# ZECTBynmo/iris-tts

Measured on AMD Instinct MI355X. Metric: audio samples/sec (22.05 kHz) on 80-mel x 1000-frame batch, higher is better.
Workload: dtype f32

## Files before the change

### iris-tts_amd/csrc/conv_mfma_bf16.h

```cpp
#pragma once
#include <hip/hip_runtime.h>
#include <stdint.h>
#include <stdlib.h>
#include <string.h>
#include "pcm_out.h"

namespace iris {
namespace b16 {

typedef __bf16 bf16x8 __attribute__((ext_vector_type(8)));
typedef __bf16 bf16x2 __attribute__((ext_vector_type(2)));
typedef float f32x2 __attribute__((ext_vector_type(2)));
typedef float f32x4 __attribute__((ext_vector_type(4)));
typedef float f32x16 __attribute__((ext_vector_type(16)));
typedef unsigned int u32x2 __attribute__((ext_vector_type(2)));
typedef unsigned int u32x4 __attribute__((ext_vector_type(4)));

#ifndef IRIS_B16_XCD_FOLD
#define IRIS_B16_XCD_FOLD 1
#endif

#ifndef IRIS_B16_UPS32_MT
#define IRIS_B16_UPS32_MT 3
#endif

enum InAct : int { IN_ACT_NONE = 0, IN_ACT_LRELU = 1, IN_ACT_MRF_LRELU = 2 };

constexpr int kMaxGroup = 4;

struct Problem {
    const void* x;
    const void* wp;
    const float* bias;
    const uint16_t* res;
    uint16_t* y;
    int ks;
    int dil;
    int pad_left;
    int reserved;
};

struct Launch {
    Problem p[kMaxGroup];
    const uint16_t* xmrf[kMaxGroup];
    int n_mrf;
    int B, L_in, L_out, C_in, C_out;
    int n_idx;
    int out_stride;
    int out_off;
    int z_is_phase;
    unsigned phase_wp_bytes;
    int in_act;
    int x_f32_cf;
    float slope;
    float inv_n_mrf;
    int nz;
    int n_co_blk;
    int Qp;
    int n_ct;
    int n_items;
    int n_share;
    int xcd_group;
    int fold_b;
    int z_in_y;
};

__device__ __forceinline__ float bf_lo(unsigned w) { return __builtin_bit_cast(float, w << 16); }
__device__ __forceinline__ float bf_hi(unsigned w) { return __builtin_bit_cast(float, w & 0xffff0000u); }
__device__ __forceinline__ unsigned pack_bf2(float lo, float hi) {
    const f32x2 v = {lo, hi};
    return __builtin_bit_cast(unsigned, __builtin_convertvector(v, bf16x2));
}
__device__ __forceinline__ float lrelu1(float v, float slope) { return v > 0.f ? v : v * slope; }

__device__ __forceinline__ __amdgpu_buffer_rsrc_t make_rsrc(const void* base, unsigned bytes) {
    return __builtin_amdgcn_make_buffer_rsrc(const_cast<void*>(base), 0, (int)bytes, 0x00020000);
}
__device__ __forceinline__ u32x4 buf_load4(__amdgpu_buffer_rsrc_t r, unsigned voff, unsigned soff) {
    return __builtin_amdgcn_raw_buffer_load_b128(r, (int)voff, (int)soff, 0);
}
__device__ __forceinline__ u32x2 buf_load2(__amdgpu_buffer_rsrc_t r, unsigned voff, unsigned soff) {
    return __builtin_amdgcn_raw_buffer_load_b64(r, (int)voff, (int)soff, 0);
}
__device__ __forceinline__ void buf_store2(u32x2 v, __amdgpu_buffer_rsrc_t r, unsigned voff, unsigned soff) {
    __builtin_amdgcn_raw_buffer_store_b64(v, r, (int)voff, (int)soff, 0);
}
constexpr unsigned kOob = 0x80000000u;

template <int CIC>
__device__ __forceinline__ void stage_window(const Launch& a, const Problem& p, char* lds, int b,
                                             int in_row0, int R, int c0) {
    constexpr int SB = CIC * 2 + 16;
    constexpr int PPR = CIC / 8;
    const int tid = threadIdx.x;
    const int L_in = a.L_in, C_in = a.C_in;
    if (!a.x_f32_cf) {
        const unsigned tensor_bytes = (unsigned)L_in * (unsigned)C_in * 2u;
        const size_t boff = (size_t)b * L_in * C_in;
        const bool mrf = a.in_act == IN_ACT_MRF_LRELU;
        const __amdgpu_buffer_rsrc_t r0 = make_rsrc((mrf ? a.xmrf[0] : (const uint16_t*)p.x) + boff, tensor_bytes);
        const __amdgpu_buffer_rsrc_t r1 = make_rsrc((mrf && a.n_mrf > 1 ? a.xmrf[1] : a.xmrf[0]) + boff, mrf && a.n_mrf > 1 ? tensor_bytes : 0u);
        const __amdgpu_buffer_rsrc_t r2 = make_rsrc((mrf && a.n_mrf > 2 ? a.xmrf[2] : a.xmrf[0]) + boff, mrf && a.n_mrf > 2 ? tensor_bytes : 0u);
        const __amdgpu_buffer_rsrc_t r3 = make_rsrc((mrf && a.n_mrf > 3 ? a.xmrf[3] : a.xmrf[0]) + boff, mrf && a.n_mrf > 3 ? tensor_bytes : 0u);
        const int total = R * PPR;
        const float slope = a.in_act == IN_ACT_NONE ? 1.f : a.slope;
        auto piece = [&](int idx, unsigned& voff, int& ldso) {
            const int r = idx / PPR, pc = idx - r * PPR;
            const int row = in_row0 + r, ci = c0 + 8 * pc;
            const bool ok = idx < total && row >= 0 && row < L_in && ci < C_in;
            voff = ok ? (unsigned)(row * C_in + ci) * 2u : kOob;
            ldso = idx < total ? r * SB + pc * 16 : -1;
        };
        if (!mrf) {
            constexpr int U = 4;
            for (int base = 0; base < total; base += 256 * U) {
                u32x4 v0[U];
                int ldso[U];
#pragma unroll
                for (int u = 0; u < U; ++u) {
                    unsigned voff;
                    piece(base + u * 256 + tid, voff, ldso[u]);
                    v0[u] = buf_load4(r0, voff, 0);
                }
#pragma unroll
                for (int u = 0; u < U; ++u) {
                    u32x4 o;
#pragma unroll
                    for (int e = 0; e < 4; ++e)
                        o[e] = pack_bf2(lrelu1(bf_lo(v0[u][e]), slope), lrelu1(bf_hi(v0[u][e]), slope));
                    if (ldso[u] >= 0) *reinterpret_cast<u32x4*>(lds + ldso[u]) = o;
                }
            }
        } else {
            constexpr int U = 2;
            for (int base = 0; base < total; base += 256 * U) {
                u32x4 v0[U], v1[U], v2[U], v3[U];
                int ldso[U];
#pragma unroll
                for (int u = 0; u < U; ++u) {
                    unsigned voff;
                    piece(base + u * 256 + tid, voff, ldso[u]);
                    v0[u] = buf_load4(r0, voff, 0);
                    v1[u] = buf_load4(r1, voff, 0);
                    v2[u] = buf_load4(r2, voff, 0);
                    v3[u] = buf_load4(r3, voff, 0);
                }
#pragma unroll
                for (int u = 0; u < U; ++u) {
                    u32x4 o;
#pragma unroll
                    for (int e = 0; e < 4; ++e) {
                        float lo = ((bf_lo(v0[u][e]) + bf_lo(v1[u][e])) + bf_lo(v2[u][e])) + bf_lo(v3[u][e]);
                        float hi = ((bf_hi(v0[u][e]) + bf_hi(v1[u][e])) + bf_hi(v2[u][e])) + bf_hi(v3[u][e]);
                        lo *= a.inv_n_mrf; hi *= a.inv_n_mrf;
                        o[e] = pack_bf2(lrelu1(lo, slope), lrelu1(hi, slope));
                    }
                    if (ldso[u] >= 0) *reinterpret_cast<u32x4*>(lds + ldso[u]) = o;
                }
            }
        }
    } else {
        const float* x = (const float*)p.x;
        const int total = R * CIC;
        for (int idx = tid; idx < total; idx += 256) {
            const int c = idx / R, r = idx - c * R;
            const int row = in_row0 + r, ci = c0 + c;
            float v = 0.f;
            if (row >= 0 && row < L_in && ci < C_in) {
                v = x[((size_t)b * C_in + ci) * L_in + row];
                if (a.in_act == IN_ACT_LRELU) v = lrelu1(v, a.slope);
            }
            const unsigned pk = pack_bf2(v, 0.f);
            *reinterpret_cast<uint16_t*>(lds + r * SB + c * 2) = (uint16_t)(pk & 0xffffu);
        }
    }
}

template <int MT, int NT, int CIC>
__device__ __forceinline__ void mma_chunk(f32x16 (&acc)[MT][NT], const char* a_lane, int dil_bytes,
                                          __amdgpu_buffer_rsrc_t wr, unsigned wvoff, unsigned q_bytes,
                                          unsigned tap_bytes, unsigned q0_bytes, int ks) {
    constexpr int QPC = CIC / 16;
    constexpr int QL = QPC == 8 ? 3 : (QPC == 4 ? 2 : (QPC == 2 ? 1 : 0));
    static_assert(QPC == 8 || QPC == 4 || QPC == 2 || QPC == 1, "CIC must be 16, 32, 64 or 128");
    constexpr int SB = CIC * 2 + 16;
    constexpr int D = (QPC == 2 && MT * NT >= 8) ? 2 : 4;
    const int NG = ks * QPC;
    auto w_soff = [&](int n) -> unsigned {
        return (unsigned)(n >> QL) * tap_bytes + q0_bytes + (unsigned)(n & (QPC - 1)) * q_bytes;
    };
    auto load_a = [&](u32x4 (&av)[MT], int n) {
        int tap = n >> QL;
        tap = tap < ks ? tap : ks - 1;
        const char* ap = a_lane + tap * dil_bytes + (n & (QPC - 1)) * 32;
#pragma unroll
        for (int m = 0; m < MT; ++m) av[m] = *reinterpret_cast<const u32x4*>(ap + m * 32 * SB);
    };
    u32x4 wv[D][NT], av[2][MT];
#pragma unroll
    for (int i = 0; i < D; ++i) {
#pragma unroll
        for (int nt = 0; nt < NT; ++nt) wv[i][nt] = buf_load4(wr, wvoff + (unsigned)nt * 1024u, w_soff(i));
        __builtin_amdgcn_sched_barrier(0);
    }
    load_a(av[0], 0);
    for (int n0 = 0; n0 < NG; n0 += D) {
#pragma unroll
        for (int i = 0; i < D; ++i) {
            const int n = n0 + i;
            load_a(av[(i + 1) & 1], n + 1);
            __builtin_amdgcn_sched_barrier(0);
#pragma unroll
            for (int nt = 0; nt < NT; ++nt)
#pragma unroll
                for (int m = 0; m < MT; ++m)
                    acc[m][nt] = __builtin_amdgcn_mfma_f32_32x32x16_bf16(
                        __builtin_bit_cast(bf16x8, wv[i][nt]), __builtin_bit_cast(bf16x8, av[i & 1][m]),
                        acc[m][nt], 0, 0, 0);
            __builtin_amdgcn_sched_barrier(0);
#pragma unroll
            for (int nt = 0; nt < NT; ++nt)
                wv[i][nt] = buf_load4(wr, wvoff + (unsigned)nt * 1024u, w_soff(n + D));
        }
    }
}

template <int WT, int WC, int MT, int NT, int CIC, int MINB>
__global__ void __launch_bounds__(256, MINB) conv_mfma_bf16_kernel(const Launch a) {
    extern __shared__ __attribute__((aligned(16))) char lds_b16[];
    char* lds = lds_b16;
    constexpr int SB = CIC * 2 + 16;
    constexpr int T_BLK = WT * MT * 32;
    const int lane = threadIdx.x & 63, wave = threadIdx.x >> 6;
    const int wt = wave / WC, wc = wave - wt * WC;
    const int lo = lane & 31, hi = lane >> 5;

    int w_item, sub;
    int b = blockIdx.y;
    if (a.xcd_group) {
        const int xcd = blockIdx.x & 7, s = blockIdx.x >> 3;
        sub = s % a.n_share;
        const int w_lin = (s / a.n_share) * 8 + xcd;
        if (w_lin >= a.n_items * (a.fold_b ? a.B : 1)) return;
        if (a.fold_b) { b = w_lin / a.n_items; w_item = w_lin - b * a.n_items; }
        else w_item = w_lin;
    } else {
        sub = blockIdx.x % a.n_share;
        w_item = blockIdx.x / a.n_share;
    }
    int tile_co, tile_t, zr;
    if (a.z_is_phase)   { zr = sub / a.n_co_blk; tile_co = sub - zr * a.n_co_blk; tile_t = w_item; }
    else if (a.z_in_y && a.fold_b) { tile_co = sub; tile_t = w_item; zr = blockIdx.y; }
    else if (a.z_in_y)  { tile_co = sub; tile_t = w_item; zr = blockIdx.y / a.B; b = blockIdx.y - zr * a.B; }
    else                { tile_co = sub; zr = w_item % a.nz; tile_t = w_item / a.nz; }
    const int z = a.z_is_phase ? zr : a.nz - 1 - zr;
    const int pz = a.z_is_phase ? 0 : z;
    Problem p = a.p[0];
    if (pz == 1) p = a.p[1];
    if (pz == 2) p = a.p[2];
    if (pz == 3) p = a.p[3];
    const int out_off = a.out_off + (a.z_is_phase ? z : 0);

    const int i0 = tile_t * T_BLK;
    const int ks = p.ks;
    const int R = T_BLK + (ks - 1) * p.dil;
    const int in_row0 = i0 - p.pad_left;
    const int ct0 = (tile_co * WC + wc) * NT;
    const bool wave_active = ct0 < a.n_ct;

    f32x16 acc[MT][NT];
#pragma unroll
    for (int nt = 0; nt < NT; ++nt)
#pragma unroll
        for (int g = 0; g < 4; ++g) {
            const int co = (ct0 + nt) * 32 + 8 * g + 4 * hi;
            const f32x4 b4 = *reinterpret_cast<const f32x4*>(p.bias + (co < a.C_out ? co : 0));
#pragma unroll
            for (int m = 0; m < MT; ++m)
#pragma unroll
                for (int e = 0; e < 4; ++e) acc[m][nt][4 * g + e] = b4[e];
        }

    const unsigned q_bytes = (unsigned)a.n_ct * 1024u;
    const unsigned tap_bytes = (unsigned)a.Qp * q_bytes;
    const char* wbase = (const char*)p.wp + (a.z_is_phase ? (size_t)z * a.phase_wp_bytes : 0);
    const __amdgpu_buffer_rsrc_t wr = make_rsrc(wbase, (unsigned)ks * tap_bytes);
    const unsigned wvoff = (unsigned)ct0 * 1024u + (unsigned)lane * 16u;
    const char* a_lane = lds + (wt * MT * 32 + lo) * SB + hi * 16;
    const int dil_bytes = p.dil * SB;

    for (int c0 = 0; c0 < a.C_in; c0 += CIC) {
        if (c0 > 0) __syncthreads();
        stage_window<CIC>(a, p, lds, b, in_row0, R, c0);
        __syncthreads();
        if (wave_active)
            mma_chunk<MT, NT, CIC>(acc, a_lane, dil_bytes, wr, wvoff, q_bytes, tap_bytes,
                                   (unsigned)(c0 >> 4) * q_bytes, ks);
    }
    __syncthreads();
    if (!wave_active) return;
    constexpr int RS = NT * 32 * 4 + 16;
    constexpr int PPRO = NT * 4;
    constexpr int NP = 2 * NT;
    char* scr = lds + wave * (32 * RS);
    const unsigned out_bytes = (unsigned)a.L_out * (unsigned)a.C_out * 2u;
    const size_t ob = (size_t)b * a.L_out * a.C_out;
    const __amdgpu_buffer_rsrc_t yr = make_rsrc(p.y + ob, out_bytes);
    const __amdgpu_buffer_rsrc_t rr = make_rsrc(p.res ? p.res + ob : p.y, p.res ? out_bytes : 0u);
    unsigned pvoff[MT][NP];
    int pscr[NP];
#pragma unroll
    for (int j = 0; j < NP; ++j) {
        const int q = j * 64 + lane;
        const int row_l = q / PPRO, pc = q - row_l * PPRO;
        pscr[j] = row_l * RS + pc * 32;
        const int co = ct0 * 32 + 8 * pc;
#pragma unroll
        for (int m = 0; m < MT; ++m) {
            const int im = i0 + (wt * MT + m) * 32 + row_l;
            const int o = im * a.out_stride + out_off;
            const bool ok = im < a.n_idx && o >= 0 && o < a.L_out && co < a.C_out;
            pvoff[m][j] = ok ? (unsigned)(o * a.C_out + co) * 2u : kOob;
        }
    }
    u32x4 resv[MT][NP];
#pragma unroll
    for (int m = 0; m < MT; ++m)
#pragma unroll
        for (int j = 0; j < NP; ++j) resv[m][j] = buf_load4(rr, pvoff[m][j], 0);
#pragma unroll
    for (int m = 0; m < MT; ++m) {
#pragma unroll
        for (int nt = 0; nt < NT; ++nt)
#pragma unroll
            for (int g = 0; g < 4; ++g) {
                f32x4 v;
#pragma unroll
                for (int e = 0; e < 4; ++e) v[e] = acc[m][nt][4 * g + e];
                *reinterpret_cast<f32x4*>(scr + lo * RS + (nt * 32 + 8 * g + 4 * hi) * 4) = v;
            }
        __builtin_amdgcn_fence(__ATOMIC_RELEASE, "wavefront");
        __builtin_amdgcn_wave_barrier();
        __builtin_amdgcn_fence(__ATOMIC_ACQUIRE, "wavefront");
        u32x4 outp[NP];
#pragma unroll
        for (int j = 0; j < NP; ++j) {
            const f32x4 lo4 = *reinterpret_cast<const f32x4*>(scr + pscr[j]);
            const f32x4 hi4 = *reinterpret_cast<const f32x4*>(scr + pscr[j] + 16);
            const u32x4 rv = resv[m][j];
            outp[j][0] = pack_bf2(lo4[0] + bf_lo(rv[0]), lo4[1] + bf_hi(rv[0]));
            outp[j][1] = pack_bf2(lo4[2] + bf_lo(rv[1]), lo4[3] + bf_hi(rv[1]));
            outp[j][2] = pack_bf2(hi4[0] + bf_lo(rv[2]), hi4[1] + bf_hi(rv[2]));
            outp[j][3] = pack_bf2(hi4[2] + bf_lo(rv[3]), hi4[3] + bf_hi(rv[3]));
        }
        __builtin_amdgcn_sched_barrier(0);
#pragma unroll
        for (int j = 0; j < NP; ++j)
            __builtin_amdgcn_raw_buffer_store_b128(outp[j], yr, (int)pvoff[m][j], 0, 0);
        asm volatile("s_nop 1");
        __builtin_amdgcn_sched_barrier(0);
#pragma unroll
        for (int j = 0; j < NP; ++j) asm volatile("" :: "v"(outp[j]));
        __builtin_amdgcn_fence(__ATOMIC_RELEASE, "wavefront");
        __builtin_amdgcn_wave_barrier();
    }
}

struct PostLaunch {
    const uint16_t* x[kMaxGroup];
    int n_in;
    const float* w;
    const float* bias;
    float* y;
    int16_t* pcm;
    unsigned* peak;
    int B, L, C, k;
    float slope, inv_n;
};

constexpr int kPostTile = 256;

template <int OUT>
__global__ void __launch_bounds__(256) conv_post_tanh_bf16_kernel(const PostLaunch a) {
    extern __shared__ __attribute__((aligned(16))) char lds_b16[];
    float* lds = reinterpret_cast<float*>(lds_b16);
    const int C = a.C, k = a.k, pad = (k - 1) / 2;
    const int S = C | 1;
    const int PPR = C / 8;
    const int b = blockIdx.y, t0 = blockIdx.x * kPostTile;
    const int R = kPostTile + k - 1;
    const unsigned tensor_bytes = (unsigned)a.L * (unsigned)C * 2u;
    const size_t boff = (size_t)b * a.L * C;
    const __amdgpu_buffer_rsrc_t r0 = make_rsrc(a.x[0] + boff, tensor_bytes);
    const __amdgpu_buffer_rsrc_t r1 = make_rsrc((a.n_in > 1 ? a.x[1] : a.x[0]) + boff, a.n_in > 1 ? tensor_bytes : 0u);
    const __amdgpu_buffer_rsrc_t r2 = make_rsrc((a.n_in > 2 ? a.x[2] : a.x[0]) + boff, a.n_in > 2 ? tensor_bytes : 0u);
    const __amdgpu_buffer_rsrc_t r3 = make_rsrc((a.n_in > 3 ? a.x[3] : a.x[0]) + boff, a.n_in > 3 ? tensor_bytes : 0u);
    const int total = R * PPR;
    for (int idx = threadIdx.x; idx < total; idx += 256) {
        const int r = idx / PPR, pc = idx - r * PPR;
        const int row = t0 - pad + r;
        const unsigned voff = (row >= 0 && row < a.L) ? (unsigned)(row * C + 8 * pc) * 2u : kOob;
        const u32x4 v0 = buf_load4(r0, voff, 0), v1 = buf_load4(r1, voff, 0), v2 = buf_load4(r2, voff, 0),
                    v3 = buf_load4(r3, voff, 0);
#pragma unroll
        for (int e = 0; e < 4; ++e) {
            float lo = ((bf_lo(v0[e]) + bf_lo(v1[e])) + bf_lo(v2[e])) + bf_lo(v3[e]);
            float hi = ((bf_hi(v0[e]) + bf_hi(v1[e])) + bf_hi(v2[e])) + bf_hi(v3[e]);
            if (a.n_in > 1) { lo *= a.inv_n; hi *= a.inv_n; }
            lds[r * S + 8 * pc + 2 * e] = lrelu1(lo, a.slope);
            lds[r * S + 8 * pc + 2 * e + 1] = lrelu1(hi, a.slope);
        }
    }
    __syncthreads();
    const int t = t0 + threadIdx.x;
    constexpr bool PEAK = OUT == pcm::OUT_F32_PEAK;
    if constexpr (!PEAK) {
        if (t >= a.L) return;
    }
    float wv = 0.f;
    if (!PEAK || t < a.L) {
        const float* __restrict__ w = a.w;
        float acc = a.bias[0];
        for (int kap = 0; kap < k; ++kap) {
            const float* row = lds + (threadIdx.x + kap) * S;
            for (int c = 0; c < C; ++c) acc = fmaf(row[c], w[kap * C + c], acc);
        }
        wv = tanhf(acc);
    }
    if constexpr (PEAK) {
        if (t < a.L) a.y[(size_t)b * a.L + t] = wv;
        pcm::block_peak_max(pcm::abs_bits(wv), a.peak + b);
    } else {
        pcm::store_sample<OUT>(a, (size_t)b * a.L + t, wv);
    }
}

inline hipError_t launch_conv_post_bf16(const PostLaunch& a, hipStream_t stream) {
    const size_t lds_bytes = (size_t)(kPostTile + a.k - 1) * (a.C | 1) * sizeof(float);
    if (lds_bytes > 160 * 1024 || (a.C & 7)) return hipErrorInvalidValue;
    dim3 grid((unsigned)((a.L + kPostTile - 1) / kPostTile), (unsigned)a.B), block(256);
    auto kfn = a.pcm ? conv_post_tanh_bf16_kernel<pcm::OUT_PCM16>
                     : (a.peak ? conv_post_tanh_bf16_kernel<pcm::OUT_F32_PEAK> : conv_post_tanh_bf16_kernel<pcm::OUT_F32>);
    return ::iris::launch_kernel_named("conv_post_tanh_bf16_kernel", kfn, grid, block, lds_bytes, stream, a);
}

inline uint16_t f32_to_bf16(float f) {
    uint32_t u;
    memcpy(&u, &f, 4);
    if ((u & 0x7fffffffu) > 0x7f800000u) return (uint16_t)((u >> 16) | 0x40u);
    u += 0x7fffu + ((u >> 16) & 1u);
    return (uint16_t)(u >> 16);
}

inline int packed_qsteps(int C_in) { return ((C_in + 63) / 64) * 4; }
inline int packed_cotiles(int C_out) { return (C_out + 31) / 32; }
inline size_t packed_conv1d_halfs(int C_in, int C_out, int ks) {
    return (size_t)ks * packed_qsteps(C_in) * packed_cotiles(C_out) * 64 * 8;
}
inline void pack_conv1d_bf16(const float* w, int C_in, int C_out, int ks, uint16_t* out) {
    const int Qp = packed_qsteps(C_in), n_ct = packed_cotiles(C_out);
    for (int kap = 0; kap < ks; ++kap)
        for (int q = 0; q < Qp; ++q)
            for (int ct = 0; ct < n_ct; ++ct)
                for (int lane = 0; lane < 64; ++lane)
                    for (int e = 0; e < 8; ++e) {
                        const int co = ct * 32 + (lane & 31);
                        const int ci = 16 * q + 8 * (lane >> 5) + e;
                        float v = 0.f;
                        if (co < C_out && ci < C_in) v = w[((size_t)co * C_in + ci) * ks + kap];
                        out[((((size_t)kap * Qp + q) * n_ct + ct) * 64 + lane) * 8 + e] = f32_to_bf16(v);
                    }
}
inline int convt_taps(int k, int u) { return (k + u - 1) / u; }
inline size_t packed_convt_phase_halfs(int C_in, int C_out, int k, int u) {
    return packed_conv1d_halfs(C_in, C_out, convt_taps(k, u));
}
inline void pack_convt_bf16(const float* w, int C_in, int C_out, int k, int u, uint16_t* out) {
    const int taps = convt_taps(k, u);
    const int Qp = packed_qsteps(C_in), n_ct = packed_cotiles(C_out);
    const size_t phase_halfs = packed_convt_phase_halfs(C_in, C_out, k, u);
    for (int ph = 0; ph < u; ++ph)
        for (int kap = 0; kap < taps; ++kap) {
            const int kk = ph + (taps - 1 - kap) * u;
            for (int q = 0; q < Qp; ++q)
                for (int ct = 0; ct < n_ct; ++ct)
                    for (int lane = 0; lane < 64; ++lane)
                        for (int e = 0; e < 8; ++e) {
                            const int co = ct * 32 + (lane & 31);
                            const int ci = 16 * q + 8 * (lane >> 5) + e;
                            float v = 0.f;
                            if (co < C_out && ci < C_in && kk < k) v = w[((size_t)ci * C_out + co) * k + kk];
                            out[ph * phase_halfs + ((((size_t)kap * Qp + q) * n_ct + ct) * 64 + lane) * 8 + e] =
                                f32_to_bf16(v);
                        }
        }
}

struct Tile { int WT, WC, MT, NT, CIC, MINB, T_BLK, CO_BLK; };

inline Tile pick_tile(int C_in, int C_out, bool phases = false) {
    Tile t;
    if (C_out <= 32) {
        t.WT = 4; t.WC = 1; t.NT = 1;
        t.MT = phases ? IRIS_B16_UPS32_MT : 3; t.MINB = 4;
    } else if (C_out <= 64) {
        t.WT = 2; t.WC = 2; t.MT = 3; t.NT = 1; t.MINB = 4;
    } else {
        t.WT = 2; t.WC = 2; t.NT = 2;
        t.MT = 2;
        t.MINB = 2;
    }
    t.CIC = (C_in <= 32 && t.NT == 1 && t.WC == 1) ? 32 : 64;
    if (C_out > 64 && C_in % 128 == 0) t.CIC = 128;
    t.T_BLK = t.WT * t.MT * 32;
    t.CO_BLK = t.WC * t.NT * 32;
    return t;
}

inline hipError_t launch_conv_bf16(Launch& a, int nz, hipStream_t stream) {
    const Tile t = pick_tile(a.C_in, a.C_out, a.z_is_phase != 0);
    a.n_co_blk = (a.C_out + t.CO_BLK - 1) / t.CO_BLK;
    a.Qp = packed_qsteps(a.C_in);
    a.n_ct = packed_cotiles(a.C_out);
    a.nz = nz;
    a.inv_n_mrf = a.n_mrf > 0 ? 1.0f / (float)a.n_mrf : 1.0f;
    int span = 0;
    const int np = a.z_is_phase ? 1 : nz;
    if (np > kMaxGroup) return hipErrorInvalidValue;
    for (int j = 0; j < np; ++j) {
        const int s = (a.p[j].ks - 1) * a.p[j].dil;
        if (s > span) span = s;
    }
    if ((double)a.L_in * a.C_in * 2.0 >= 2147483648.0 || (double)a.L_out * a.C_out * 2.0 >= 2147483648.0)
        return hipErrorInvalidValue;
    if (!a.x_f32_cf && (a.C_in & 7)) return hipErrorInvalidValue;
    if (a.C_out & 3) return hipErrorInvalidValue;
    const size_t window_bytes = (size_t)(t.T_BLK + span) * (t.CIC * 2 + 16);
    const size_t scratch_bytes = (size_t)4 * 32 * (t.NT * 32 * 4 + 16);
    const size_t lds_bytes = window_bytes > scratch_bytes ? window_bytes : scratch_bytes;
    if (lds_bytes > 160 * 1024) return hipErrorInvalidValue;
    const int n_t = (a.n_idx + t.T_BLK - 1) / t.T_BLK;
    a.z_in_y = !a.z_is_phase && nz > 1 && (long long)a.B * nz <= 65535;
    a.n_items = (a.z_is_phase || a.z_in_y) ? n_t : n_t * nz;
    a.n_share = a.z_is_phase ? a.n_co_blk * nz : a.n_co_blk;
    a.fold_b = IRIS_B16_XCD_FOLD;
    const long long items_all = (long long)a.n_items * (a.fold_b ? a.B : 1);
    const long long gx_grouped = ((items_all + 7) / 8) * 8 * a.n_share;
    a.xcd_group = a.n_share > 1 && items_all >= 64 && gx_grouped < 0x7fffffffLL;
    const long long gx = a.xcd_group ? gx_grouped : (long long)a.n_items * a.n_share;
    if (gx > 0x7fffffffLL) return hipErrorInvalidValue;
    a.fold_b = a.fold_b && a.xcd_group;
    const unsigned gy = a.fold_b ? (unsigned)(a.z_in_y ? nz : 1) : (unsigned)(a.z_in_y ? a.B * nz : a.B);
    dim3 grid((unsigned)gx, gy, 1u), block(256);
#define IRIS_B16_LAUNCH(...)                                                                      \
    do {                                                                                          \
        auto kfn = __VA_ARGS__;                                                                   \
        { const hipError_t e__ = ::iris::launch_kernel_named(#__VA_ARGS__, kfn, grid, block, lds_bytes, stream, a); if (e__ != hipSuccess) return e__; } \
        return hipSuccess;                                                                        \
    } while (0)
#define IRIS_B16_CASE(WT_, WC_, MT_, NT_, CIC_, MINB_)                                            \
    if (t.WT == WT_ && t.WC == WC_ && t.MT == MT_ && t.NT == NT_ && t.CIC == CIC_ && t.MINB == MINB_) \
        IRIS_B16_LAUNCH(conv_mfma_bf16_kernel<WT_, WC_, MT_, NT_, CIC_, MINB_>)
    IRIS_B16_CASE(4, 1, 3, 1, 32, 4); IRIS_B16_CASE(4, 1, 3, 1, 64, 4);
#if IRIS_B16_UPS32_MT != 3
    IRIS_B16_CASE(4, 1, IRIS_B16_UPS32_MT, 1, 32, 4); IRIS_B16_CASE(4, 1, IRIS_B16_UPS32_MT, 1, 64, 4);
#endif
    IRIS_B16_CASE(2, 2, 3, 1, 64, 4); IRIS_B16_CASE(2, 2, 2, 2, 64, 2); IRIS_B16_CASE(2, 2, 2, 2, 128, 2);
#undef IRIS_B16_CASE
#undef IRIS_B16_LAUNCH
    return hipErrorInvalidValue;
}

}
}
```

### iris-tts_amd/csrc/conv_mfma_f32s.h

```cpp
#pragma once
#include <vector>

#include "conv_mfma_bf16.h"

namespace iris {
namespace s3 {

using b16::bf16x8;
using b16::f32x4;
using b16::f32x16;
using b16::u32x2;
using b16::u32x4;
using b16::pack_bf2;
using b16::bf_lo;
using b16::bf_hi;
using b16::lrelu1;
using b16::make_rsrc;
using b16::buf_load4;
using b16::kOob;

constexpr int kMaxGroup = 4;

struct Problem {
    const float* x;
    const void* wp;
    const float* bias;
    const float* res;
    float* y;
    int ks, dil, pad_left, reserved;
};

struct Launch {
    Problem p[kMaxGroup];
    int B, L, C;
    float slope;
    int nz;
    int n_co_blk, Qp, n_ct;
    unsigned plane_bytes[kMaxGroup];
    int C_in;
    int L_in;
    int n_idx;
    int out_stride;
    int out_off;
    int z_is_phase;
    unsigned phase_bytes;
    float* sum_y;
    float sum_div;
};

template <int CIC>
__device__ __forceinline__ void stage_window(const Launch& a, const Problem& p, char* lds_hi, char* lds_mid, int b,
                                             int in_row0, int R, int c0) {
    constexpr int SB = CIC * 2 + 16;
    constexpr int PPR = CIC / 4;
    const int tid = threadIdx.x;
    const int Lin = a.L_in ? a.L_in : a.L, Cin = a.C_in ? a.C_in : a.C;
    const unsigned tensor_bytes = (unsigned)Lin * (unsigned)Cin * 4u;
    const __amdgpu_buffer_rsrc_t xr = make_rsrc(p.x + (size_t)b * Lin * Cin, tensor_bytes);
    const int total = R * PPR;
    constexpr int U = 4;
    for (int base = 0; base < total; base += 256 * U) {
        u32x4 v[U];
#pragma unroll
        for (int u = 0; u < U; ++u) {
            const int idx = base + u * 256 + tid;
            const int r = idx / PPR, pc = idx - r * PPR;
            const int row = in_row0 + r;
            const bool ok = idx < total && row >= 0 && row < Lin;
            v[u] = buf_load4(xr, ok ? (unsigned)(row * Cin + c0 + 4 * pc) * 4u : kOob, 0);
        }
#pragma unroll
        for (int u = 0; u < U; ++u) {
            const int idx = base + u * 256 + tid;
            const int r = idx / PPR, pc = idx - r * PPR;
            float f[4], h[4];
#pragma unroll
            for (int e = 0; e < 4; ++e) {
                const unsigned w = v[u][e];
                f[e] = lrelu1(__builtin_bit_cast(float, w), a.slope);
            }
            u32x2 hi, mid;
            hi[0] = pack_bf2(f[0], f[1]); hi[1] = pack_bf2(f[2], f[3]);
            h[0] = bf_lo(hi[0]); h[1] = bf_hi(hi[0]); h[2] = bf_lo(hi[1]); h[3] = bf_hi(hi[1]);
            mid[0] = pack_bf2(f[0] - h[0], f[1] - h[1]); mid[1] = pack_bf2(f[2] - h[2], f[3] - h[3]);
            if (idx < total) {
                *reinterpret_cast<u32x2*>(lds_hi + r * SB + pc * 8) = hi;
                *reinterpret_cast<u32x2*>(lds_mid + r * SB + pc * 8) = mid;
            }
        }
    }
}

template <int WT, int WC, int MT, int NT, int CIC, int MINB, bool ZS>
__global__ void __launch_bounds__(256, MINB) conv_mfma_f32s_kernel(const Launch a) {
    extern __shared__ __attribute__((aligned(16))) char lds_s3[];
    char* lds = lds_s3;
    constexpr int SB = CIC * 2 + 16;
    constexpr int QPC = CIC / 16;
    constexpr int QL = QPC == 4 ? 2 : 1;
    static_assert(QPC == 4 || QPC == 2, "CIC must be 32 or 64");
    constexpr int T_BLK = WT * MT * 32;
    constexpr int D = 2;
    const int lane = threadIdx.x & 63, wave = threadIdx.x >> 6;
    const int wt = wave / WC, wc = wave - wt * WC;
    const int lo = lane & 31, hi = lane >> 5;

    const int sub = blockIdx.x % a.n_co_blk, item = blockIdx.x / a.n_co_blk;
    const int nzp = ZS ? 1 : a.nz;
    const int zr = item % nzp, tile_t = item / nzp;
    const int b = blockIdx.y;
    const int i0 = tile_t * T_BLK;
    constexpr int RS = NT * 32 * 4 + 16;
    constexpr int PPRO = NT * 8;
    constexpr int NP = 4 * NT;
    f32x4 msum[ZS ? MT : 1][ZS ? NP : 1];
    const int n_pass = ZS ? a.nz : 1;
  for (int zi = 0; zi < n_pass; ++zi) {
    const int z = ZS ? zi : (a.z_is_phase ? zr : a.nz - 1 - zr);
    Problem p = a.p[0];
    unsigned plane_bytes = a.plane_bytes[0];
    if (!a.z_is_phase) {
        if (z == 1) { p = a.p[1]; plane_bytes = a.plane_bytes[1]; }
        if (z == 2) { p = a.p[2]; plane_bytes = a.plane_bytes[2]; }
        if (z == 3) { p = a.p[3]; plane_bytes = a.plane_bytes[3]; }
    }
    const int Cin = a.C_in ? a.C_in : a.C;
    const int ostride = a.out_stride ? a.out_stride : 1;
    const int ooff = a.out_off + (a.z_is_phase ? z : 0);
    if (ZS && zi > 0) __syncthreads();
    const int ks = p.ks;
    const int span = (ks - 1) * p.dil;
    const int R = T_BLK + span;
    const int in_row0 = i0 - p.pad_left;
    const int ct0 = (sub * WC + wc) * NT;
    char* const lds_hi = lds;
    char* const lds_mid = lds + R * SB;

    f32x16 acc[MT][NT];
#pragma unroll
    for (int m = 0; m < MT; ++m)
#pragma unroll
        for (int nt = 0; nt < NT; ++nt)
#pragma unroll
            for (int r = 0; r < 16; ++r) acc[m][nt][r] = 0.f;

    const unsigned q_bytes = (unsigned)a.n_ct * 1024u;
    const unsigned tap_bytes = (unsigned)a.Qp * q_bytes;
    const unsigned phase_off = a.z_is_phase ? (unsigned)z * a.phase_bytes : 0u;
    const __amdgpu_buffer_rsrc_t wr = make_rsrc((const char*)p.wp + phase_off, plane_bytes + (unsigned)ks * tap_bytes);
    const unsigned wvoff = (unsigned)ct0 * 1024u + (unsigned)lane * 16u;
    const int a_off = (wt * MT * 32 + lo) * SB + hi * 16;
    const int dil_bytes = p.dil * SB;
    const int NG = ks * QPC;

    for (int c0 = 0; c0 < Cin; c0 += CIC) {
        if (c0 > 0) __syncthreads();
        stage_window<CIC>(a, p, lds_hi, lds_mid, b, in_row0, R, c0);
        __syncthreads();
        const unsigned q0_bytes = (unsigned)(c0 >> 4) * q_bytes;
        auto w_soff = [&](int n) -> unsigned {
            return (unsigned)(n >> QL) * tap_bytes + q0_bytes + (unsigned)(n & (QPC - 1)) * q_bytes;
        };
        auto load_w = [&](u32x4 (&wh)[NT], u32x4 (&wm)[NT], int n) {
            const bool in = n < NG;
            const unsigned so = w_soff(in ? n : 0);
#pragma unroll
            for (int nt = 0; nt < NT; ++nt) {
                wh[nt] = buf_load4(wr, in ? wvoff + (unsigned)nt * 1024u : kOob, so);
                wm[nt] = buf_load4(wr, in ? wvoff + (unsigned)nt * 1024u : kOob, so + plane_bytes);
            }
        };
        auto load_a = [&](u32x4 (&ah)[MT], u32x4 (&am)[MT], int n) {
            int tap = n >> QL;
            tap = tap < ks ? tap : ks - 1;
            const int off = a_off + tap * dil_bytes + (n & (QPC - 1)) * 32;
#pragma unroll
            for (int m = 0; m < MT; ++m) {
                ah[m] = *reinterpret_cast<const u32x4*>(lds_hi + off + m * 32 * SB);
                am[m] = *reinterpret_cast<const u32x4*>(lds_mid + off + m * 32 * SB);
            }
        };
        u32x4 wh[D][NT], wm[D][NT], ah[2][MT], am[2][MT];
#pragma unroll
        for (int i = 0; i < D; ++i) {
            load_w(wh[i], wm[i], i);
            __builtin_amdgcn_sched_barrier(0);
        }
        load_a(ah[0], am[0], 0);
        for (int n0 = 0; n0 < NG; n0 += D) {
#pragma unroll
            for (int i = 0; i < D; ++i) {
                const int n = n0 + i;
                load_a(ah[(i + 1) & 1], am[(i + 1) & 1], n + 1);
                __builtin_amdgcn_sched_barrier(0);
#pragma unroll
                for (int nt = 0; nt < NT; ++nt)
#pragma unroll
                    for (int m = 0; m < MT; ++m) {
                        acc[m][nt] = __builtin_amdgcn_mfma_f32_32x32x16_bf16(
                            __builtin_bit_cast(bf16x8, wm[i][nt]), __builtin_bit_cast(bf16x8, ah[i & 1][m]), acc[m][nt], 0, 0, 0);
                        acc[m][nt] = __builtin_amdgcn_mfma_f32_32x32x16_bf16(
                            __builtin_bit_cast(bf16x8, wh[i][nt]), __builtin_bit_cast(bf16x8, am[i & 1][m]), acc[m][nt], 0, 0, 0);
                        acc[m][nt] = __builtin_amdgcn_mfma_f32_32x32x16_bf16(
                            __builtin_bit_cast(bf16x8, wh[i][nt]), __builtin_bit_cast(bf16x8, ah[i & 1][m]), acc[m][nt], 0, 0, 0);
                    }
                __builtin_amdgcn_sched_barrier(0);
                load_w(wh[i], wm[i], n + D);
            }
        }
    }

    __syncthreads();
    char* const scr = lds + wave * (32 * RS);
    const unsigned tensor_bytes = (unsigned)a.L * (unsigned)a.C * 4u;
    const size_t ob = (size_t)b * a.L * a.C;
    const __amdgpu_buffer_rsrc_t yr = make_rsrc((ZS ? a.sum_y : p.y) + ob, tensor_bytes);
    const __amdgpu_buffer_rsrc_t rr = make_rsrc(p.res ? p.res + ob : p.y, p.res ? tensor_bytes : 0u);
    unsigned pv[NP];
    int pscr[NP];
#pragma unroll
    for (int j = 0; j < NP; ++j) {
        const int q = j * 64 + lane;
        const int row_l = q / PPRO, pc = q - row_l * PPRO;
        pscr[j] = row_l * RS + pc * 16;
        pv[j] = (unsigned)(((i0 + wt * MT * 32 + row_l) * ostride + ooff) * a.C + ct0 * 32 + 4 * pc) * 4u;
    }
    f32x4 bias4[NT][4];
#pragma unroll
    for (int nt = 0; nt < NT; ++nt)
#pragma unroll
        for (int g = 0; g < 4; ++g) bias4[nt][g] = *reinterpret_cast<const f32x4*>(p.bias + (ct0 + nt) * 32 + 8 * g + 4 * hi);
#pragma unroll
    for (int m = 0; m < MT; ++m) {
        const unsigned msoff = (unsigned)(m * 32 * ostride * a.C) * 4u;
        u32x4 resv[NP];
#pragma unroll
        for (int j = 0; j < NP; ++j) resv[j] = buf_load4(rr, pv[j] + msoff, 0);
#pragma unroll
        for (int nt = 0; nt < NT; ++nt)
#pragma unroll
            for (int g = 0; g < 4; ++g) {
                f32x4 v;
#pragma unroll
                for (int e = 0; e < 4; ++e) v[e] = acc[m][nt][4 * g + e] + bias4[nt][g][e];
                *reinterpret_cast<f32x4*>(scr + lo * RS + (nt * 32 + 8 * g + 4 * hi) * 4) = v;
            }
        __builtin_amdgcn_fence(__ATOMIC_RELEASE, "wavefront");
        __builtin_amdgcn_wave_barrier();
        __builtin_amdgcn_fence(__ATOMIC_ACQUIRE, "wavefront");
        u32x4 outp[NP];
#pragma unroll
        for (int j = 0; j < NP; ++j) {
            const f32x4 v = *reinterpret_cast<const f32x4*>(scr + pscr[j]);
#pragma unroll
            for (int e = 0; e < 4; ++e) {
                const unsigned rw = resv[j][e];
                float o = v[e] + __builtin_bit_cast(float, rw);
                if constexpr (ZS) {
                    o = zi == 0 ? o : msum[m][j][e] + o;
                    msum[m][j][e] = o;
                    if (zi == n_pass - 1) o = o / a.sum_div;
                }
                outp[j][e] = __builtin_bit_cast(unsigned, o);
            }
        }
        __builtin_amdgcn_sched_barrier(0);
        if (!ZS || zi == n_pass - 1) {
#pragma unroll
            for (int j = 0; j < NP; ++j)
                __builtin_amdgcn_raw_buffer_store_b128(outp[j], yr, (int)(pv[j] + msoff), 0, 0);
        }
        asm volatile("s_nop 1");
        __builtin_amdgcn_sched_barrier(0);
#pragma unroll
        for (int j = 0; j < NP; ++j) asm volatile("" :: "v"(outp[j]));
        __builtin_amdgcn_fence(__ATOMIC_RELEASE, "wavefront");
        __builtin_amdgcn_wave_barrier();
    }
  }
}

inline size_t packed_plane_halfs(int C_in, int C_out, int ks) { return b16::packed_conv1d_halfs(C_in, C_out, ks); }
inline void pack_conv1d_split(const float* w, int C_in, int C_out, int ks, uint16_t* out) {
    const size_t n = (size_t)C_out * C_in * ks;
    std::vector<float> hi(n), mid(n);
    for (size_t i = 0; i < n; ++i) {
        const uint16_t h = b16::f32_to_bf16(w[i]);
        uint32_t u = (uint32_t)h << 16;
        float hf;
        memcpy(&hf, &u, 4);
        hi[i] = hf;
        mid[i] = w[i] - hf;
    }
    b16::pack_conv1d_bf16(hi.data(), C_in, C_out, ks, out);
    b16::pack_conv1d_bf16(mid.data(), C_in, C_out, ks, out + packed_plane_halfs(C_in, C_out, ks));
}

inline size_t packed_convt_plane_halfs(int C_in, int C_out, int k, int u) { return b16::packed_convt_phase_halfs(C_in, C_out, k, u) * u; }
inline void pack_convt_split(const float* w, int C_in, int C_out, int k, int u, uint16_t* out) {
    const size_t n = (size_t)C_in * C_out * k;
    std::vector<float> hi(n), mid(n);
    for (size_t i = 0; i < n; ++i) {
        const uint16_t h = b16::f32_to_bf16(w[i]);
        uint32_t bits = (uint32_t)h << 16;
        float hf;
        memcpy(&hf, &bits, 4);
        hi[i] = hf;
        mid[i] = w[i] - hf;
    }
    b16::pack_convt_bf16(hi.data(), C_in, C_out, k, u, out);
    b16::pack_convt_bf16(mid.data(), C_in, C_out, k, u, out + packed_convt_plane_halfs(C_in, C_out, k, u));
}

struct Tile { int WT, WC, MT, NT, CIC, MINB, T_BLK, CO_BLK; };
inline Tile pick_tile(int C) {
    Tile t;
    if (C <= 32)      { t.WT = 4; t.WC = 1; t.MT = 2; t.NT = 1; t.CIC = 32; }
    else if (C <= 64) { t.WT = 2; t.WC = 2; t.MT = 2; t.NT = 1; t.CIC = 64; }
    else              { t.WT = 2; t.WC = 2; t.MT = 2; t.NT = 2; t.CIC = 64; }
    t.MINB = 2;
    t.T_BLK = t.WT * t.MT * 32;
    t.CO_BLK = t.WC * t.NT * 32;
    return t;
}

inline bool applicable(const Launch& a, int nz) {
    if (nz < 1 || (!a.z_is_phase && nz > kMaxGroup) || a.C < 32 || (a.C & 31)) return false;
    const Tile t = pick_tile(a.C);
    const int Cin = a.C_in ? a.C_in : a.C, Lin = a.L_in ? a.L_in : a.L;
    if (Cin % t.CIC || a.C % t.CO_BLK) return false;
    if ((double)a.L * a.C * 4.0 >= 2147483648.0 - 4194304.0 || (double)Lin * Cin * 4.0 >= 2147483648.0 - 4194304.0)
        return false;
    return true;
}

inline hipError_t launch(Launch& a, int nz, hipStream_t stream) {
    Tile t = pick_tile(a.C);
    a.n_co_blk = a.C / t.CO_BLK;
    const int Cin = a.C_in ? a.C_in : a.C;
    const int n_rows = a.n_idx ? a.n_idx : a.L;
    a.Qp = b16::packed_qsteps(Cin);
    a.n_ct = b16::packed_cotiles(a.C);
    a.nz = nz;
    int span = 0;
    for (int j = 0; j < (a.z_is_phase ? 1 : nz); ++j) {
        const int s = (a.p[j].ks - 1) * a.p[j].dil;
        if (s > span) span = s;
        if (!a.z_is_phase) a.plane_bytes[j] = (unsigned)(packed_plane_halfs(a.C, a.C, a.p[j].ks) * 2);
    }
    const bool zs = a.sum_y != nullptr;
    a.sum_div = (float)nz;
    static const int n_cu = [] { int dev = 0, n = 256; (void)hipGetDevice(&dev);
                                 (void)hipDeviceGetAttribute(&n, hipDeviceAttributeMultiprocessorCount, dev); return n > 0 ? n : 256; }();
    const long long blocks2 = (long long)((n_rows + t.T_BLK - 1) / t.T_BLK) * (zs ? 1 : nz) * a.n_co_blk * a.B;
    if (2 * blocks2 < 5LL * n_cu) { t.MT = 1; t.T_BLK = t.WT * 32; }
    const int SB = t.CIC * 2 + 16;
    const size_t window = 2 * (size_t)(t.T_BLK + span) * SB;
    const size_t scratch = (size_t)4 * 32 * (t.NT * 32 * 4 + 16);
    const size_t lds_bytes = window > scratch ? window : scratch;
    if (lds_bytes > 160 * 1024) return hipErrorInvalidValue;
    const int n_t = (n_rows + t.T_BLK - 1) / t.T_BLK;
    dim3 grid((unsigned)(n_t * (zs ? 1 : nz) * a.n_co_blk), (unsigned)a.B, 1u), block(256);
#define IRIS_S3_LAUNCH(...)                                                                       \
    do {                                                                                          \
        auto kfn = __VA_ARGS__;                                                                   \
         \
        { const hipError_t e__ = ::iris::launch_kernel_named(#__VA_ARGS__, kfn, grid, block, lds_bytes, stream, a); if (e__ != hipSuccess) return e__; } \
        return hipSuccess;                                                                        \
    } while (0)
#define IRIS_S3_CASE(WT_, WC_, NT_, CIC_)                                                         \
    if (t.WT == WT_ && t.WC == WC_ && t.NT == NT_) {                                              \
        if (zs) { if (t.MT == 1) IRIS_S3_LAUNCH(conv_mfma_f32s_kernel<WT_, WC_, 1, NT_, CIC_, 2, true>);    \
                  else           IRIS_S3_LAUNCH(conv_mfma_f32s_kernel<WT_, WC_, 2, NT_, CIC_, 2, true>); }  \
        else    { if (t.MT == 1) IRIS_S3_LAUNCH(conv_mfma_f32s_kernel<WT_, WC_, 1, NT_, CIC_, 2, false>);   \
                  else           IRIS_S3_LAUNCH(conv_mfma_f32s_kernel<WT_, WC_, 2, NT_, CIC_, 2, false>); } \
    }
    IRIS_S3_CASE(4, 1, 1, 32)
    IRIS_S3_CASE(2, 2, 1, 64)
    IRIS_S3_CASE(2, 2, 2, 64)
#undef IRIS_S3_CASE
#undef IRIS_S3_LAUNCH
    return hipErrorInvalidValue;
}

}
}
```

### iris-tts_amd/csrc/convt_mfma_bf16.h

```cpp
#pragma once
#include "conv_mfma_bf16.h"

namespace iris {
namespace b16 {

#ifndef IRIS_CONVT_GEMM_B16_DEFAULT
#define IRIS_CONVT_GEMM_B16_DEFAULT 1
#endif

#ifndef IRIS_CONVT_B16_WIDE_A
#define IRIS_CONVT_B16_WIDE_A 1
#endif

struct ConvtLaunch {
    const uint16_t* x[3];
    const void* wp;
    const float* bias;
    uint16_t* y;
    int B, L_in, L_out, C_in, C_out;
    int u, out_off;
    int n_idx;
    int Qp, n_ct;
    unsigned phase_bytes;
    int n_row_tiles;
    int n_items;
    int n_col_blk;
    int xcd_order;
    int jobs_per_xcd;
    int in_act;
    float slope, inv_n;
};

template <int MT, int NT, int WR, int WC, int CIC, int NIN, int MINB>
__global__ void __launch_bounds__(256, MINB) convt_mfma_bf16_kernel(const ConvtLaunch a) {
    static_assert(NIN == 1 || NIN == 3, "one input tensor, or the three branch outputs of the previous stage");
    static_assert(WR * WC == 4, "four waves per block");
    extern __shared__ __attribute__((aligned(16))) char lds_b16[];
    char* const lds = lds_b16;
    constexpr int SB = CIC * 2 + 16;
    constexpr int PPR = CIC / 8;
    constexpr int QPC = CIC / 16;
    constexpr int R_BLK = WR * MT * 32;
    constexpr int WIN = R_BLK + 1;
    constexpr int NQ = (WIN * PPR + 255) / 256;
    constexpr int RPI = 256 / PPR;
    constexpr int NG = 2 * QPC;
    constexpr int LPG = (NQ + NG - 1) / NG;
    constexpr int DB = 4;
    static_assert(DB <= QPC && NG > DB, "the ring reaches into tap 0 of the next phase only");
    constexpr int RS = NT * 32 * 4 + 16;
    constexpr int PPRO = NT * 4;
    constexpr int NP = 2 * NT;

    const int tid = threadIdx.x, lane = tid & 63, wave = tid >> 6;
    const int wr = wave / WC, wc = wave - wr * WC;
    const int lo = lane & 31, hi = lane >> 5;
    const int C = a.C_in;
    const int n_chunks = C / CIC;
    const float slope = a.in_act == IN_ACT_NONE ? 1.f : a.slope;
    const unsigned in_bytes = (unsigned)a.L_in * (unsigned)C * 2u;
    const unsigned out_bytes = (unsigned)a.L_out * (unsigned)a.C_out * 2u;
    const unsigned q_bytes = (unsigned)a.n_ct * 1024u;
    const unsigned tap_bytes = (unsigned)a.Qp * q_bytes;
    const __amdgpu_buffer_rsrc_t wrs = make_rsrc(a.wp, (unsigned)a.u * a.phase_bytes);
    char* const scr = lds + WIN * SB + wave * (32 * RS);
    float* const lds_bias = reinterpret_cast<float*>(lds + WIN * SB + 4 * (32 * RS));

    for (int i = tid; i < (a.C_out >> 2); i += 256)
        *reinterpret_cast<f32x4*>(lds_bias + 4 * i) = *reinterpret_cast<const f32x4*>(a.bias + 4 * i);

    const int r_lane = tid / PPR, p_lane = tid - r_lane * PPR;
    const unsigned row_stride = (unsigned)(RPI * C) * 2u;
    char* const lds_wr = lds + r_lane * SB + p_lane * 16;
    u32x4 st[NIN][NQ];
    auto stage_vbase = [&](int in_row0, int c0) -> unsigned {
        return (unsigned)((in_row0 + r_lane) * C + c0 + 8 * p_lane) * 2u;
    };
    auto stage_load_one = [&](int i, size_t x_off, unsigned bytes, unsigned vbase) {
        const unsigned voff = r_lane + i * RPI < WIN ? vbase + (unsigned)i * row_stride : kOob;
#pragma unroll
        for (int t = 0; t < NIN; ++t) st[t][i] = buf_load4(make_rsrc(a.x[t] + x_off, bytes), voff, 0);
    };
    auto stage_write_all = [&]() {
#pragma unroll
        for (int i = 0; i < NQ; ++i)
            if (r_lane + i * RPI < WIN) {
                u32x4 o;
#pragma unroll
                for (int e = 0; e < 4; ++e) {
                    if constexpr (NIN == 3) {
                        float l = ((bf_lo(st[0][i][e]) + bf_lo(st[1][i][e])) + bf_lo(st[2][i][e])) + 0.f;
                        float h = ((bf_hi(st[0][i][e]) + bf_hi(st[1][i][e])) + bf_hi(st[2][i][e])) + 0.f;
                        l *= a.inv_n; h *= a.inv_n;
                        o[e] = pack_bf2(lrelu1(l, slope), lrelu1(h, slope));
                    } else {
                        o[e] = pack_bf2(lrelu1(bf_lo(st[0][i][e]), slope), lrelu1(bf_hi(st[0][i][e]), slope));
                    }
                }
                *reinterpret_cast<u32x4*>(lds_wr + i * RPI * SB) = o;
            }
    };

    struct Tile { size_t x_off, y_off; int i0, gct0; unsigned wvoff[NT]; };
    const int xmul = a.xcd_order ? 8 : 1;
    const int xcd = a.xcd_order ? (int)(blockIdx.x & 7) : 0;
    const int slot = a.xcd_order ? (int)(blockIdx.x >> 3) : (int)blockIdx.x;
    const int slots = a.xcd_order ? (int)(gridDim.x >> 3) : (int)gridDim.x;
    auto job_valid = [&](int job) { return job < a.jobs_per_xcd && (job / a.n_col_blk) * xmul + xcd < a.n_items; };
    auto make_tile = [&](int job) {
        Tile t;
        const int il = job / a.n_col_blk, cb = job - il * a.n_col_blk;
        const int item = il * xmul + xcd;
        const int b = item / a.n_row_tiles, rt = item - b * a.n_row_tiles;
        t.x_off = (size_t)b * a.L_in * C;
        t.y_off = (size_t)b * a.L_out * a.C_out;
        t.i0 = rt * R_BLK;
        t.gct0 = (cb * WC + wc) * NT;
#pragma unroll
        for (int nt = 0; nt < NT; ++nt) {
            const int gct = t.gct0 + nt;
            const int ph = gct / a.n_ct, ct = gct - ph * a.n_ct;
            t.wvoff[nt] = (unsigned)ph * a.phase_bytes + (unsigned)(ct * 64 + lane) * 16u;
        }
        return t;
    };

    const char* a_lane = lds + (wr * MT * 32 + lo) * SB + hi * 16;
    f32x16 acc[MT][NT];
    u32x4 bw[DB + 1][NT];

    int job = slot;
    if (!job_valid(job)) return;
    Tile t = make_tile(job);
    {
        const unsigned vb0 = stage_vbase(t.i0 - 1, 0);
#pragma unroll
        for (int i = 0; i < NQ; ++i) stage_load_one(i, t.x_off, in_bytes, vb0);
#pragma unroll
        for (int d = 0; d < DB; ++d)
#pragma unroll
            for (int nt = 0; nt < NT; ++nt) bw[d][nt] = buf_load4(wrs, t.wvoff[nt], (unsigned)d * q_bytes);
        stage_write_all();
        __syncthreads();
    }
    for (;;) {
        const int job_next = job + slots;
        const bool more = job_valid(job_next);
        const Tile tn = make_tile(more ? job_next : job);
#pragma unroll
        for (int nt = 0; nt < NT; ++nt) {
            const int gct = t.gct0 + nt;
            const int ct = gct % a.n_ct;
#pragma unroll
            for (int g = 0; g < 4; ++g) {
                const f32x4 b4 = *reinterpret_cast<const f32x4*>(lds_bias + ct * 32 + 8 * g + 4 * hi);
#pragma unroll
                for (int m = 0; m < MT; ++m)
#pragma unroll
                    for (int e = 0; e < 4; ++e) acc[m][nt][4 * g + e] = b4[e];
            }
        }

        for (int chunk = 0; chunk < n_chunks; ++chunk) {
            const bool last = chunk + 1 == n_chunks;
            const bool has_next = !last || more;
            const Tile& tq = last ? tn : t;
            const int cq = last ? 0 : chunk + 1;
            const unsigned in_bytes_n = has_next ? in_bytes : 0u;
            const unsigned vbn = stage_vbase(tq.i0 - 1, cq * CIC);
            const unsigned wsoff0 = (unsigned)(chunk * QPC) * q_bytes;
            const unsigned wsoffn = (unsigned)(cq * QPC) * q_bytes;
            auto a_ptr = [&](int n) { return a_lane + (n / QPC) * SB + (n % QPC) * 32; };
            auto b_load = [&](int n, int nt) {
                if (n < NG)
                    return buf_load4(wrs, t.wvoff[nt], wsoff0 + (unsigned)(n / QPC) * tap_bytes + (unsigned)(n % QPC) * q_bytes);
                return buf_load4(wrs, has_next ? tq.wvoff[nt] : kOob, wsoffn + (unsigned)(n - NG) * q_bytes);
            };
            u32x4 av[2][MT];
#pragma unroll
            for (int m = 0; m < MT; ++m) av[0][m] = *reinterpret_cast<const u32x4*>(a_ptr(0) + m * 32 * SB);
#pragma unroll
            for (int n = 0; n < NG; ++n) {
#pragma unroll
                for (int l = 0; l < LPG; ++l)
                    if (n * LPG + l < NQ) stage_load_one(n * LPG + l, tq.x_off, in_bytes_n, vbn);
#pragma unroll
                for (int nt = 0; nt < NT; ++nt) bw[(n + DB) % (DB + 1)][nt] = b_load(n + DB, nt);
                if (n + 1 < NG) {
#pragma unroll
                    for (int m = 0; m < MT; ++m)
                        av[(n + 1) & 1][m] = *reinterpret_cast<const u32x4*>(a_ptr(n + 1) + m * 32 * SB);
                }
#pragma unroll
                for (int nt = 0; nt < NT; ++nt)
#pragma unroll
                    for (int m = 0; m < MT; ++m)
                        acc[m][nt] = __builtin_amdgcn_mfma_f32_32x32x16_bf16(
                            __builtin_bit_cast(bf16x8, bw[n % (DB + 1)][nt]), __builtin_bit_cast(bf16x8, av[n & 1][m]),
                            acc[m][nt], 0, 0, 0);
                __builtin_amdgcn_sched_barrier(0);
            }
            {
                u32x4 tmp[DB][NT];
#pragma unroll
                for (int d = 0; d < DB; ++d)
#pragma unroll
                    for (int nt = 0; nt < NT; ++nt) tmp[d][nt] = bw[(NG + d) % (DB + 1)][nt];
#pragma unroll
                for (int d = 0; d < DB; ++d)
#pragma unroll
                    for (int nt = 0; nt < NT; ++nt) bw[d][nt] = tmp[d][nt];
            }
            if (last) {
                const __amdgpu_buffer_rsrc_t yr = make_rsrc(a.y + t.y_off, out_bytes);
                int prow[NP], pph[NP], pco[NP], pscr[NP];
#pragma unroll
                for (int j = 0; j < NP; ++j) {
                    const int q = j * 64 + lane;
                    const int row_l = q / PPRO, pc = q - row_l * PPRO;
                    const int gct = t.gct0 + (pc >> 2);
                    const int ph = gct / a.n_ct, ct = gct - ph * a.n_ct;
                    prow[j] = row_l; pph[j] = ph; pco[j] = ct * 32 + 8 * (pc & 3);
                    pscr[j] = row_l * RS + pc * 32;
                }
#pragma unroll
                for (int m = 0; m < MT; ++m) {
#pragma unroll
                    for (int nt = 0; nt < NT; ++nt)
#pragma unroll
                        for (int g = 0; g < 4; ++g) {
                            f32x4 v;
#pragma unroll
                            for (int e = 0; e < 4; ++e) v[e] = acc[m][nt][4 * g + e];
                            *reinterpret_cast<f32x4*>(scr + lo * RS + (nt * 32 + 8 * g + 4 * hi) * 4) = v;
                        }
                    __builtin_amdgcn_fence(__ATOMIC_RELEASE, "wavefront");
                    __builtin_amdgcn_wave_barrier();
                    __builtin_amdgcn_fence(__ATOMIC_ACQUIRE, "wavefront");
                    u32x4 outp[NP];
                    unsigned pvoff[NP];
#pragma unroll
                    for (int j = 0; j < NP; ++j) {
                        const f32x4 lo4 = *reinterpret_cast<const f32x4*>(scr + pscr[j]);
                        const f32x4 hi4 = *reinterpret_cast<const f32x4*>(scr + pscr[j] + 16);
                        outp[j][0] = pack_bf2(lo4[0] + 0.f, lo4[1] + 0.f);
                        outp[j][1] = pack_bf2(lo4[2] + 0.f, lo4[3] + 0.f);
                        outp[j][2] = pack_bf2(hi4[0] + 0.f, hi4[1] + 0.f);
                        outp[j][3] = pack_bf2(hi4[2] + 0.f, hi4[3] + 0.f);
                        const int i = t.i0 + (wr * MT + m) * 32 + prow[j];
                        const int o = i * a.u + a.out_off + pph[j];
                        const bool ok = i < a.n_idx && o >= 0 && o < a.L_out;
                        pvoff[j] = ok ? (unsigned)(o * a.C_out + pco[j]) * 2u : kOob;
                    }
                    __builtin_amdgcn_sched_barrier(0);
#pragma unroll
                    for (int j = 0; j < NP; ++j)
                        __builtin_amdgcn_raw_buffer_store_b128(outp[j], yr, (int)pvoff[j], 0, 0);
                    asm volatile("s_nop 1");
                    __builtin_amdgcn_sched_barrier(0);
#pragma unroll
                    for (int j = 0; j < NP; ++j) asm volatile("" :: "v"(outp[j]));
                    __builtin_amdgcn_fence(__ATOMIC_RELEASE, "wavefront");
                    __builtin_amdgcn_wave_barrier();
                }
            }
            if (has_next) {
                __syncthreads();
                stage_write_all();
                __syncthreads();
            }
        }
        if (!more) break;
        job = job_next;
        t = tn;
    }
}

#ifndef IRIS_KERNELS_ONLY
struct ConvtTile { int MT, NT, WR, WC, CIC, MINB; };

inline bool convt_gemm_b16_applicable(int C_in, int C_out, int k, int u, int L_in, int L_out, int B, int n_in, float slope) {
    if (!IRIS_CONVT_GEMM_B16_DEFAULT) return false;
    if (u < 1 || k != 2 * u) return false;
    if ((C_in & 63) || (C_out & 31)) return false;
    if (n_in != 1 && n_in != 3) return false;
    if (((u * (C_out / 32)) & 1)) return false;
    if ((uint64_t)L_in * C_in * 2u >= 0x7fffffffull || (uint64_t)L_out * C_out * 2u >= 0x7fffffffull) return false;
    if ((uint64_t)u * packed_convt_phase_halfs(C_in, C_out, k, u) * 2u >= 0x7fffffffull) return false;
    if ((uint64_t)(L_in + 1 + 255) * (uint64_t)B >= 0x3fffffffull) return false;
    (void)slope;
    return true;
}

inline hipError_t launch_convt_gemm_b16(ConvtLaunch& a, int k, hipStream_t stream) {
    a.n_idx = a.L_in + 1;
    a.out_off = -(k - a.u) / 2;
    a.Qp = packed_qsteps(a.C_in);
    a.n_ct = packed_cotiles(a.C_out);
    a.phase_bytes = (unsigned)(packed_convt_phase_halfs(a.C_in, a.C_out, k, a.u) * 2);
    const int n_cols32 = a.u * a.n_ct;
    const int n_cu = device_cu_count();
    const int CIC = (a.C_out > 64 && a.C_in % 128 == 0) ? 128 : 64;
    ConvtTile t;
    auto blocks_of = [&](int rows, int cols32) { return (long long)((a.n_idx + rows - 1) / rows) * (n_cols32 / cols32) * a.B; };
    if (CIC == 128) {
        if (IRIS_CONVT_B16_WIDE_A && (n_cols32 & 7) == 0 && blocks_of(64, 8) >= 2LL * n_cu) t = ConvtTile{2, 2, 1, 4, 128, 2};
        else if ((n_cols32 & 3) == 0) t = ConvtTile{2, 1, 1, 4, 128, 3};
        else return hipErrorInvalidValue;
    } else {
        if ((n_cols32 & 3) == 0) t = ConvtTile{2, 1, 1, 4, 64, 3};
        else t = ConvtTile{2, 1, 2, 2, 64, 3};
    }
    const int rows = t.WR * t.MT * 32;
    a.n_row_tiles = (a.n_idx + rows - 1) / rows;
    a.n_col_blk = n_cols32 / (t.WC * t.NT);
    const long long n_items = (long long)a.n_row_tiles * a.B;
    if (n_items * a.n_col_blk > 0x3fffffffLL) return hipErrorInvalidValue;
    a.n_items = (int)n_items;
    const long long items8 = ((n_items + 7) / 8) * 8;
    a.xcd_order = a.n_col_blk > 1 && (items8 - n_items) * 8 <= n_items;
    const int xm = a.xcd_order ? 8 : 1;
    a.jobs_per_xcd = a.xcd_order ? (int)(items8 / 8) * a.n_col_blk : (int)(n_items * a.n_col_blk);
    a.inv_n = a.in_act == IN_ACT_MRF_LRELU ? 1.0f / 3.0f : 1.0f;
    const bool three = a.in_act == IN_ACT_MRF_LRELU;
    const size_t lds_bytes = (size_t)(rows + 1) * (CIC * 2 + 16) + (size_t)4 * 32 * (t.NT * 128 + 16) + (size_t)a.C_out * 4;
    long long per_cu = (!three && t.NT == 1) ? 4 : t.MINB;
    { const long long by_lds = (long long)(160 * 1024) / (long long)lds_bytes; if (by_lds < per_cu) per_cu = by_lds; }
    if (per_cu < 1) return hipErrorInvalidValue;
    const long long cap = per_cu * (n_cu / xm);
    long long g = a.jobs_per_xcd < cap ? a.jobs_per_xcd : cap;
    if (g < 1) g = 1;
    const long long rounds = (a.jobs_per_xcd + g - 1) / g;
    g = (a.jobs_per_xcd + rounds - 1) / rounds;
    g *= xm;
    dim3 grid((unsigned)g, 1u, 1u), block(256);
#define IRIS_CONVT_B16_CASE(MT_, NT_, WR_, WC_, CIC_, MINB_)                                                                   \
    if (t.MT == MT_ && t.NT == NT_ && t.WR == WR_ && t.CIC == CIC_) {                                                         \
        if (three) return ::iris::launch_kernel_named("convt_mfma_bf16_kernel<" #MT_ ", " #NT_ ", " #WR_ ", " #WC_ ", " #CIC_ ", 3>", \
                              convt_mfma_bf16_kernel<MT_, NT_, WR_, WC_, CIC_, 3, MINB_>, grid, block, lds_bytes, stream, a);  \
        return ::iris::launch_kernel_named("convt_mfma_bf16_kernel<" #MT_ ", " #NT_ ", " #WR_ ", " #WC_ ", " #CIC_ ", 1>",      \
                              convt_mfma_bf16_kernel<MT_, NT_, WR_, WC_, CIC_, 1, MINB_>, grid, block, lds_bytes, stream, a);  \
    }
    IRIS_CONVT_B16_CASE(2, 2, 1, 4, 128, 2)
    IRIS_CONVT_B16_CASE(2, 1, 1, 4, 128, 3)
    IRIS_CONVT_B16_CASE(2, 1, 1, 4, 64, 3)
    IRIS_CONVT_B16_CASE(2, 1, 2, 2, 64, 3)
#undef IRIS_CONVT_B16_CASE
    return hipErrorInvalidValue;
}

inline hipError_t launch_convt_bf16(Launch& a, int k, int u, hipStream_t stream) {
    const int n_in = a.in_act == IN_ACT_MRF_LRELU ? a.n_mrf : 1;
    if (!a.x_f32_cf && convt_gemm_b16_applicable(a.C_in, a.C_out, k, u, a.L_in, a.L_out, a.B, n_in, a.slope)) {
        ConvtLaunch g; memset(&g, 0, sizeof(g));
        if (a.in_act == IN_ACT_MRF_LRELU) { g.x[0] = a.xmrf[0]; g.x[1] = a.xmrf[1]; g.x[2] = a.xmrf[2]; }
        else { g.x[0] = (const uint16_t*)a.p[0].x; g.x[1] = g.x[0]; g.x[2] = g.x[0]; }
        g.wp = a.p[0].wp; g.bias = a.p[0].bias; g.y = a.p[0].y;
        g.B = a.B; g.L_in = a.L_in; g.L_out = a.L_out; g.C_in = a.C_in; g.C_out = a.C_out;
        g.u = u; g.in_act = a.in_act; g.slope = a.slope;
        const hipError_t e = launch_convt_gemm_b16(g, k, stream);
        if (e != hipErrorInvalidValue) return e;
    }
    return launch_conv_bf16(a, u, stream);
}
#endif

}
}
```

### iris-tts_amd/csrc/mrf_pair_bf16.h

```cpp
#pragma once
#include <stdio.h>
#include "conv_mfma_bf16.h"
#ifndef IRIS_B16_RES_EARLY
#define IRIS_B16_RES_EARLY 1
#endif

#ifndef IRIS_B16_RING_TAIL_GUARD
#define IRIS_B16_RING_TAIL_GUARD 1
#endif
#ifndef IRIS_B16_PAIR_SUM_DEFAULT
#define IRIS_B16_PAIR_SUM_DEFAULT 1
#endif
#ifndef IRIS_B16_SUM32_MT
#define IRIS_B16_SUM32_MT 3
#endif
#ifndef IRIS_B16_SUM64_MT
#define IRIS_B16_SUM64_MT 3
#endif
#ifndef IRIS_B16_SUM32_MINB
#define IRIS_B16_SUM32_MINB 2
#endif
#ifndef IRIS_B16_SUM64_MINB
#define IRIS_B16_SUM64_MINB 2
#endif

namespace iris {
namespace b16 {

struct PairProblem {
    const uint16_t* x;
    const void* w1;
    const void* w2;
    const float* b1;
    const float* b2;
    uint16_t* y;
    int ks;
    int dil;
};

struct PairLaunch {
    PairProblem p[kMaxGroup];
    int B, L, C;
    float slope;
    int nz;
    int Qp, n_ct;
    int n_jobs;
    int jobs_per_xcd;
    int bias_off;
    void* sum_y;
    int sum_f32;
    float inv_n;
};

constexpr int kPairSpanMax = 50;

__device__ __forceinline__ float lrelu_max(float v, float slope) { return fmaxf(v, v * slope); }

template <int NT, int CIC, int D>
__device__ __forceinline__ void ring_request(u32x4 (&wv)[D][NT], __amdgpu_buffer_rsrc_t wr, unsigned wvoff,
                                             unsigned q_bytes, unsigned tap_bytes) {
    constexpr int QPC = CIC / 16;
    constexpr int QL = QPC == 8 ? 3 : (QPC == 4 ? 2 : (QPC == 2 ? 1 : 0));
#pragma unroll
    for (int i = 0; i < D; ++i) {
#pragma unroll
        for (int nt = 0; nt < NT; ++nt)
            wv[i][nt] = buf_load4(wr, wvoff + (unsigned)nt * 1024u, (unsigned)(i >> QL) * tap_bytes + (unsigned)(i & (QPC - 1)) * q_bytes);
        __builtin_amdgcn_sched_barrier(0);
    }
}

template <int MT, int NT, int CIC, int D>
__device__ __forceinline__ void ring_mma_loop(f32x16 (&acc)[MT][NT], u32x4 (&wv)[D][NT], const char* a_lane, int dil_bytes,
                                              __amdgpu_buffer_rsrc_t wr, unsigned wvoff, unsigned q_bytes,
                                              unsigned tap_bytes, int ks) {
    constexpr int QPC = CIC / 16;
    constexpr int QL = QPC == 8 ? 3 : (QPC == 4 ? 2 : (QPC == 2 ? 1 : 0));
    constexpr int SB = CIC * 2 + 16;
    const int NG = ks * QPC;
    auto w_soff = [&](int n) -> unsigned { return (unsigned)(n >> QL) * tap_bytes + (unsigned)(n & (QPC - 1)) * q_bytes; };
    auto load_a = [&](u32x4 (&av)[MT], int n) {
        int tap = n >> QL;
        tap = tap < ks ? tap : ks - 1;
        const char* ap = a_lane + tap * dil_bytes + (n & (QPC - 1)) * 32;
#pragma unroll
        for (int m = 0; m < MT; ++m) av[m] = *reinterpret_cast<const u32x4*>(ap + m * 32 * SB);
    };
    u32x4 av[2][MT];
    load_a(av[0], 0);
    auto group = [&](int i, int n) {
        load_a(av[(i + 1) & 1], n + 1);
        __builtin_amdgcn_sched_barrier(0);
#pragma unroll
        for (int nt = 0; nt < NT; ++nt)
#pragma unroll
            for (int m = 0; m < MT; ++m)
                acc[m][nt] = __builtin_amdgcn_mfma_f32_32x32x16_bf16(
                    __builtin_bit_cast(bf16x8, wv[i][nt]), __builtin_bit_cast(bf16x8, av[i & 1][m]), acc[m][nt], 0, 0, 0);
        __builtin_amdgcn_sched_barrier(0);
#pragma unroll
        for (int nt = 0; nt < NT; ++nt)
            wv[i][nt] = buf_load4(wr, wvoff + (unsigned)nt * 1024u, w_soff(n + D));
    };
    constexpr bool kTail = IRIS_B16_RING_TAIL_GUARD && (QPC % D) != 0;
    const int NG_main = kTail ? (NG / D) * D : NG;
    int n0 = 0;
    for (; n0 < NG_main; n0 += D) {
#pragma unroll
        for (int i = 0; i < D; ++i) group(i, n0 + i);
    }
    if constexpr (kTail) {
        if (n0 < NG) {
#pragma unroll
            for (int i = 0; i < QPC; ++i) group(i, n0 + i);
        }
    }
}

template <int WT, int WC, int MT, int NT, int C, int MINB>
__global__ void __launch_bounds__(256, MINB) mrf_pair_bf16_kernel(const PairLaunch a) {
    extern __shared__ __attribute__((aligned(16))) char lds_pair[];
    char* lds = lds_pair;
    static_assert(WT * WC == 4 && WC * NT * 32 == C, "a block owns all C channels");
    constexpr int SB = C * 2 + 16;
    constexpr int M = WT * MT * 32;
    constexpr int PPR = C / 8;
    constexpr int NQ = ((M + kPairSpanMax) * PPR + 255) / 256;
    constexpr int D = 4;
    const int lane = threadIdx.x & 63, wave = threadIdx.x >> 6;
    const int wt = wave / WC, wc = wave - wt * WC;
    const int lo = lane & 31, hi = lane >> 5;

    const int xcd = blockIdx.x & 7, slot = blockIdx.x >> 3;
    const int job = xcd * a.jobs_per_xcd + slot;
    if (job >= a.n_jobs) return;
    const int tile = job / a.nz, zr = job - tile * a.nz;
    const int z = a.nz - 1 - zr;
    PairProblem p = a.p[0];
    if (z == 1) p = a.p[1];
    if (z == 2) p = a.p[2];
    if (z == 3) p = a.p[3];
    const int ks = p.ks, dil = p.dil;
    const int h2 = (ks - 1) / 2, h1 = dil * (ks - 1) / 2;
    const int T_OUT = M - (ks - 1);
    const int o0 = tile * T_OUT;
    const int L = a.L;
    if (o0 >= L) return;
    const int b = blockIdx.y;
    const int ct0 = wc * NT;

    const unsigned tensor_bytes = (unsigned)L * (unsigned)C * 2u;
    const size_t item = (size_t)b * L * C;
    const unsigned q_bytes = (unsigned)a.n_ct * 1024u;
    const unsigned tap_bytes = (unsigned)a.Qp * q_bytes;
    const unsigned wvoff = (unsigned)ct0 * 1024u + (unsigned)lane * 16u;
    const char* a_lane = lds + (wt * MT * 32 + lo) * SB + hi * 16;
    const __amdgpu_buffer_rsrc_t xr = make_rsrc(p.x + item, tensor_bytes);
    const __amdgpu_buffer_rsrc_t wr1 = make_rsrc(p.w1, (unsigned)ks * tap_bytes);
    const __amdgpu_buffer_rsrc_t wr2 = make_rsrc(p.w2, (unsigned)ks * tap_bytes);

    f32x16 acc[MT][NT];
    auto load_bias = [&](f32x4 (&bias4)[NT][4], const float* bptr) {
#pragma unroll
        for (int nt = 0; nt < NT; ++nt)
#pragma unroll
            for (int g = 0; g < 4; ++g) bias4[nt][g] = *reinterpret_cast<const f32x4*>(bptr + (ct0 + nt) * 32 + 8 * g + 4 * hi);
    };
    auto init_acc = [&](const f32x4 (&bias4)[NT][4]) {
#pragma unroll
        for (int m = 0; m < MT; ++m)
#pragma unroll
            for (int nt = 0; nt < NT; ++nt)
#pragma unroll
                for (int r = 0; r < 16; ++r) acc[m][nt][r] = bias4[nt][r >> 2][r & 3];
    };

    constexpr int RS = NT * 32 * 4 + 16;
    constexpr int PPRO = NT * 4;
    constexpr int NP = 2 * NT;
    const __amdgpu_buffer_rsrc_t yr = make_rsrc(p.y + item, tensor_bytes);
    const __amdgpu_buffer_rsrc_t rr = make_rsrc(p.x + item, tensor_bytes);
    unsigned pvoff[MT][NP];
    int pscr[NP];
    auto geometry = [&](int lane_) {
#pragma unroll
        for (int j = 0; j < NP; ++j) {
            const int q = j * 64 + lane_;
            const int row_l = q / PPRO, pc = q - row_l * PPRO;
            pscr[j] = row_l * RS + pc * 32;
            const int co = ct0 * 32 + 8 * pc;
#pragma unroll
            for (int m = 0; m < MT; ++m) {
                const int im = (wt * MT + m) * 32 + row_l;
                const int o = o0 + im;
                pvoff[m][j] = (im < T_OUT && o < L) ? (unsigned)(o * C + co) * 2u : kOob;
            }
        }
    };
    constexpr int RBUF = IRIS_B16_RES_EARLY ? MT : 2;
    u32x4 resv[RBUF][NP];
    if constexpr (IRIS_B16_RES_EARLY) geometry(lane);
    f32x4 bias4[NT][4];
    load_bias(bias4, p.b1);
    u32x4 wv[D][NT];
    ring_request<NT, C, D>(wv, wr1, wvoff, q_bytes, tap_bytes);
    {
        const int in_row0 = o0 - h2 - h1, R = M + (ks - 1) * dil, total = R * PPR;
        u32x4 v[NQ];
#pragma unroll
        for (int u = 0; u < NQ; ++u) {
            const int idx = u * 256 + (int)threadIdx.x;
            const int r = idx / PPR, pc = idx & (PPR - 1);
            const int row = in_row0 + r;
            const bool ok = idx < total && row >= 0 && row < L;
            v[u] = buf_load4(xr, ok ? (unsigned)(row * C + 8 * pc) * 2u : kOob, 0);
        }
#pragma unroll
        for (int u = 0; u < NQ; ++u) {
            const int idx = u * 256 + (int)threadIdx.x;
            const int r = idx / PPR, pc = idx & (PPR - 1);
            u32x4 o;
#pragma unroll
            for (int e = 0; e < 4; ++e) {
                const unsigned w = v[u][e];
                o[e] = pack_bf2(lrelu_max(bf_lo(w), a.slope), lrelu_max(bf_hi(w), a.slope));
            }
            if (idx < total) *reinterpret_cast<u32x4*>(lds + r * SB + pc * 16) = o;
        }
    }
    if constexpr (IRIS_B16_RES_EARLY) {
#pragma unroll
        for (int m = 0; m < MT; ++m)
#pragma unroll
            for (int j = 0; j < NP; ++j) resv[m][j] = buf_load4(rr, pvoff[m][j], 0);
    }
    __syncthreads();
    init_acc(bias4);
    ring_mma_loop<MT, NT, C, D>(acc, wv, a_lane, dil * SB, wr1, wvoff, q_bytes, tap_bytes, ks);
    ring_request<NT, C, D>(wv, wr2, wvoff, q_bytes, tap_bytes);
    load_bias(bias4, p.b2);
    __syncthreads();
#pragma unroll
    for (int m = 0; m < MT; ++m) {
        const int row_l = (wt * MT + m) * 32 + lo;
        const int row_g = o0 - h2 + row_l;
        const unsigned keep = (row_g >= 0 && row_g < L) ? 0xffffffffu : 0u;
#pragma unroll
        for (int nt = 0; nt < NT; ++nt)
#pragma unroll
            for (int g = 0; g < 4; ++g) {
                u32x2 o;
#pragma unroll
                for (int e2 = 0; e2 < 2; ++e2) {
                    const unsigned t = pack_bf2(acc[m][nt][4 * g + 2 * e2], acc[m][nt][4 * g + 2 * e2 + 1]);
                    o[e2] = pack_bf2(lrelu_max(bf_lo(t), a.slope), lrelu_max(bf_hi(t), a.slope)) & keep;
                }
                *reinterpret_cast<u32x2*>(lds + row_l * SB + ((ct0 + nt) * 32 + 8 * g + 4 * hi) * 2) = o;
            }
    }
    {
        int lane2 = lane;
        if constexpr (IRIS_B16_RES_EARLY) asm volatile("" : "+v"(lane2));
        geometry(lane2);
    }
    if constexpr (!IRIS_B16_RES_EARLY) {
#pragma unroll
        for (int j = 0; j < NP; ++j) resv[0][j] = buf_load4(rr, pvoff[0][j], 0);
    }
    __syncthreads();
    init_acc(bias4);
    ring_mma_loop<MT, NT, C, D>(acc, wv, a_lane, SB, wr2, wvoff, q_bytes, tap_bytes, ks);
    __syncthreads();
    char* scr = lds + wave * (32 * RS);
#pragma unroll
    for (int m = 0; m < MT; ++m) {
        if (!IRIS_B16_RES_EARLY && m + 1 < MT) {
#pragma unroll
            for (int j = 0; j < NP; ++j) resv[(m + 1) & 1][j] = buf_load4(rr, pvoff[m + 1][j], 0);
        }
#pragma unroll
        for (int nt = 0; nt < NT; ++nt)
#pragma unroll
            for (int g = 0; g < 4; ++g) {
                f32x4 v;
#pragma unroll
                for (int e = 0; e < 4; ++e) v[e] = acc[m][nt][4 * g + e];
                *reinterpret_cast<f32x4*>(scr + lo * RS + (nt * 32 + 8 * g + 4 * hi) * 4) = v;
            }
        __builtin_amdgcn_fence(__ATOMIC_RELEASE, "wavefront");
        __builtin_amdgcn_wave_barrier();
        __builtin_amdgcn_fence(__ATOMIC_ACQUIRE, "wavefront");
        u32x4 outp[NP];
#pragma unroll
        for (int j = 0; j < NP; ++j) {
            const f32x4 lo4 = *reinterpret_cast<const f32x4*>(scr + pscr[j]);
            const f32x4 hi4 = *reinterpret_cast<const f32x4*>(scr + pscr[j] + 16);
            const u32x4 rv = resv[IRIS_B16_RES_EARLY ? m : (m & 1)][j];
            outp[j][0] = pack_bf2(lo4[0] + bf_lo(rv[0]), lo4[1] + bf_hi(rv[0]));
            outp[j][1] = pack_bf2(lo4[2] + bf_lo(rv[1]), lo4[3] + bf_hi(rv[1]));
            outp[j][2] = pack_bf2(hi4[0] + bf_lo(rv[2]), hi4[1] + bf_hi(rv[2]));
            outp[j][3] = pack_bf2(hi4[2] + bf_lo(rv[3]), hi4[3] + bf_hi(rv[3]));
        }
        __builtin_amdgcn_sched_barrier(0);
#pragma unroll
        for (int j = 0; j < NP; ++j)
            __builtin_amdgcn_raw_buffer_store_b128(outp[j], yr, (int)pvoff[m][j], 0, 0);
        asm volatile("s_nop 1");
        __builtin_amdgcn_sched_barrier(0);
#pragma unroll
        for (int j = 0; j < NP; ++j) asm volatile("" :: "v"(outp[j]));
        __builtin_amdgcn_fence(__ATOMIC_RELEASE, "wavefront");
        __builtin_amdgcn_wave_barrier();
    }
}

template <int WT, int WC, int MT, int NT, int C, int MINB>
__global__ void __launch_bounds__(256, MINB) mrf_pair_bf16_sum_kernel(const PairLaunch a) {
    extern __shared__ __attribute__((aligned(16))) char lds_pair[];
    char* lds = lds_pair;
    static_assert(WT * WC == 4 && WC * NT * 32 == C, "a block owns all C channels");
    constexpr int SB = C * 2 + 16;
    constexpr int M = WT * MT * 32;
    constexpr int PPR = C / 8;
    constexpr int NQ = ((M + kPairSpanMax) * PPR + 255) / 256;
    constexpr int D = 4;
    constexpr int NZ = 3;
    const int lane = threadIdx.x & 63, wave = threadIdx.x >> 6;
    const int wt = wave / WC, wc = wave - wt * WC;
    const int lo = lane & 31, hi = lane >> 5;
    const int xcd = blockIdx.x & 7, slot = blockIdx.x >> 3;
    const int tile = xcd * a.jobs_per_xcd + slot;
    if (tile >= a.n_jobs) return;
    int kmax = a.p[0].ks;
    if (a.p[1].ks > kmax) kmax = a.p[1].ks;
    if (a.p[2].ks > kmax) kmax = a.p[2].ks;
    const int T_OUT = M - (kmax - 1);
    const int o0 = tile * T_OUT;
    const int L = a.L;
    if (o0 >= L) return;
    const int b = blockIdx.y;
    const int ct0 = wc * NT;
    const unsigned tensor_bytes = (unsigned)L * (unsigned)C * 2u;
    const size_t item = (size_t)b * L * C;
    const unsigned q_bytes = (unsigned)a.n_ct * 1024u;
    const unsigned tap_bytes = (unsigned)a.Qp * q_bytes;
    const unsigned wvoff = (unsigned)ct0 * 1024u + (unsigned)lane * 16u;
    const char* a_lane = lds + (wt * MT * 32 + lo) * SB + hi * 16;

    constexpr int RS = NT * 32 * 4 + 16;
    constexpr int PPRO = NT * 4;
    constexpr int NP = 2 * NT;
    unsigned pvoff[MT][NP];
    int pscr[NP];
#pragma unroll
    for (int j = 0; j < NP; ++j) {
        const int q = j * 64 + lane;
        const int row_l = q / PPRO, pc = q - row_l * PPRO;
        pscr[j] = row_l * RS + pc * 32;
        const int co = ct0 * 32 + 8 * pc;
#pragma unroll
        for (int m = 0; m < MT; ++m) {
            const int im = (wt * MT + m) * 32 + row_l;
            const int o = o0 + im;
            pvoff[m][j] = (im < T_OUT && o < L) ? (unsigned)(o * C + co) * 2u : kOob;
        }
    }
    float sum[MT][NP][8];
    f32x16 acc[MT][NT];
    auto load_bias = [&](f32x4 (&bias4)[NT][4], const float* bptr) {
#pragma unroll
        for (int nt = 0; nt < NT; ++nt)
#pragma unroll
            for (int g = 0; g < 4; ++g) bias4[nt][g] = *reinterpret_cast<const f32x4*>(bptr + (ct0 + nt) * 32 + 8 * g + 4 * hi);
    };
    auto init_acc = [&](const f32x4 (&bias4)[NT][4]) {
#pragma unroll
        for (int m = 0; m < MT; ++m)
#pragma unroll
            for (int nt = 0; nt < NT; ++nt)
#pragma unroll
                for (int r = 0; r < 16; ++r) acc[m][nt][r] = bias4[nt][r >> 2][r & 3];
    };
    char* scr = lds + wave * (32 * RS);

#pragma unroll
    for (int z = 0; z < NZ; ++z) {
        asm volatile("; bf16 summing pair, branch %0" :: "n"(z) : "memory");
        const PairProblem& p = a.p[z];
        const int ks = p.ks, dil = p.dil;
        const int h2 = (ks - 1) / 2, h1 = dil * (ks - 1) / 2;
        const __amdgpu_buffer_rsrc_t xr = make_rsrc(p.x + item, tensor_bytes);
        const __amdgpu_buffer_rsrc_t wr1 = make_rsrc(p.w1, (unsigned)ks * tap_bytes);
        const __amdgpu_buffer_rsrc_t wr2 = make_rsrc(p.w2, (unsigned)ks * tap_bytes);
        if (z > 0) __syncthreads();
        f32x4 bias4[NT][4];
        load_bias(bias4, p.b1);
        u32x4 wv[D][NT];
        ring_request<NT, C, D>(wv, wr1, wvoff, q_bytes, tap_bytes);
        {
            const int in_row0 = o0 - h2 - h1, R = M + (ks - 1) * dil, total = R * PPR;
            u32x4 v[NQ];
#pragma unroll
            for (int u = 0; u < NQ; ++u) {
                const int idx = u * 256 + (int)threadIdx.x;
                const int r = idx / PPR, pc = idx & (PPR - 1);
                const int row = in_row0 + r;
                const bool ok = idx < total && row >= 0 && row < L;
                v[u] = buf_load4(xr, ok ? (unsigned)(row * C + 8 * pc) * 2u : kOob, 0);
            }
#pragma unroll
            for (int u = 0; u < NQ; ++u) {
                const int idx = u * 256 + (int)threadIdx.x;
                const int r = idx / PPR, pc = idx & (PPR - 1);
                u32x4 o;
#pragma unroll
                for (int e = 0; e < 4; ++e) {
                    const unsigned w = v[u][e];
                    o[e] = pack_bf2(lrelu_max(bf_lo(w), a.slope), lrelu_max(bf_hi(w), a.slope));
                }
                if (idx < total) *reinterpret_cast<u32x4*>(lds + r * SB + pc * 16) = o;
            }
        }
        __syncthreads();
        init_acc(bias4);
        ring_mma_loop<MT, NT, C, D>(acc, wv, a_lane, dil * SB, wr1, wvoff, q_bytes, tap_bytes, ks);
        ring_request<NT, C, D>(wv, wr2, wvoff, q_bytes, tap_bytes);
        load_bias(bias4, p.b2);
        __syncthreads();
#pragma unroll
        for (int m = 0; m < MT; ++m) {
            const int row_l = (wt * MT + m) * 32 + lo;
            const int row_g = o0 - h2 + row_l;
            const unsigned keep = (row_g >= 0 && row_g < L) ? 0xffffffffu : 0u;
#pragma unroll
            for (int nt = 0; nt < NT; ++nt)
#pragma unroll
                for (int g = 0; g < 4; ++g) {
                    u32x2 o;
#pragma unroll
                    for (int e2 = 0; e2 < 2; ++e2) {
                        const unsigned t = pack_bf2(acc[m][nt][4 * g + 2 * e2], acc[m][nt][4 * g + 2 * e2 + 1]);
                        o[e2] = pack_bf2(lrelu_max(bf_lo(t), a.slope), lrelu_max(bf_hi(t), a.slope)) & keep;
                    }
                    *reinterpret_cast<u32x2*>(lds + row_l * SB + ((ct0 + nt) * 32 + 8 * g + 4 * hi) * 2) = o;
                }
        }
        const __amdgpu_buffer_rsrc_t rr = make_rsrc(p.x + item, tensor_bytes);
        constexpr int RB = (MT * NT > 3) ? 1 : 2;
        u32x4 resv[RB][NP];
        if (RB == 2) {
#pragma unroll
            for (int j = 0; j < NP; ++j) resv[0][j] = buf_load4(rr, pvoff[0][j], 0);
        }
        __syncthreads();
        init_acc(bias4);
        ring_mma_loop<MT, NT, C, D>(acc, wv, a_lane, SB, wr2, wvoff, q_bytes, tap_bytes, ks);
        __syncthreads();
#pragma unroll
        for (int m = 0; m < MT; ++m) {
            if (RB == 2) {
                if (m + 1 < MT) {
#pragma unroll
                    for (int j = 0; j < NP; ++j) resv[(m + 1) % RB][j] = buf_load4(rr, pvoff[m + 1][j], 0);
                }
            } else {
#pragma unroll
                for (int j = 0; j < NP; ++j) resv[0][j] = buf_load4(rr, pvoff[m][j], 0);
            }
#pragma unroll
            for (int nt = 0; nt < NT; ++nt)
#pragma unroll
                for (int g = 0; g < 4; ++g) {
                    f32x4 v;
#pragma unroll
                    for (int e = 0; e < 4; ++e) v[e] = acc[m][nt][4 * g + e];
                    *reinterpret_cast<f32x4*>(scr + lo * RS + (nt * 32 + 8 * g + 4 * hi) * 4) = v;
                }
            __builtin_amdgcn_fence(__ATOMIC_RELEASE, "wavefront");
            __builtin_amdgcn_wave_barrier();
            __builtin_amdgcn_fence(__ATOMIC_ACQUIRE, "wavefront");
#pragma unroll
            for (int j = 0; j < NP; ++j) {
                const f32x4 lo4 = *reinterpret_cast<const f32x4*>(scr + pscr[j]);
                const f32x4 hi4 = *reinterpret_cast<const f32x4*>(scr + pscr[j] + 16);
                const u32x4 rv = resv[m % RB][j];
                unsigned yp[4];
                yp[0] = pack_bf2(lo4[0] + bf_lo(rv[0]), lo4[1] + bf_hi(rv[0]));
                yp[1] = pack_bf2(lo4[2] + bf_lo(rv[1]), lo4[3] + bf_hi(rv[1]));
                yp[2] = pack_bf2(hi4[0] + bf_lo(rv[2]), hi4[1] + bf_hi(rv[2]));
                yp[3] = pack_bf2(hi4[2] + bf_lo(rv[3]), hi4[3] + bf_hi(rv[3]));
#pragma unroll
                for (int e = 0; e < 4; ++e) {
                    if (z == 0) { sum[m][j][2 * e] = bf_lo(yp[e]); sum[m][j][2 * e + 1] = bf_hi(yp[e]); }
                    else        { sum[m][j][2 * e] = sum[m][j][2 * e] + bf_lo(yp[e]); sum[m][j][2 * e + 1] = sum[m][j][2 * e + 1] + bf_hi(yp[e]); }
                }
            }
            __builtin_amdgcn_fence(__ATOMIC_RELEASE, "wavefront");
            __builtin_amdgcn_wave_barrier();
        }
    }
    if (a.sum_f32) {
        const __amdgpu_buffer_rsrc_t yr = make_rsrc((float*)a.sum_y + item, tensor_bytes * 2u);
#pragma unroll
        for (int m = 0; m < MT; ++m)
#pragma unroll
            for (int j = 0; j < NP; ++j) {
                u32x4 o0v, o1v;
#pragma unroll
                for (int e = 0; e < 4; ++e) {
                    o0v[e] = __builtin_bit_cast(unsigned, (sum[m][j][e] + 0.f) * a.inv_n);
                    o1v[e] = __builtin_bit_cast(unsigned, (sum[m][j][4 + e] + 0.f) * a.inv_n);
                }
                const unsigned vo = pvoff[m][j] == kOob ? kOob : pvoff[m][j] * 2u;
                __builtin_amdgcn_raw_buffer_store_b128(o0v, yr, (int)vo, 0, 0);
                __builtin_amdgcn_raw_buffer_store_b128(o1v, yr, (int)vo, 16, 0);
            }
    } else {
        const __amdgpu_buffer_rsrc_t yr = make_rsrc((uint16_t*)a.sum_y + item, tensor_bytes);
#pragma unroll
        for (int m = 0; m < MT; ++m)
#pragma unroll
            for (int j = 0; j < NP; ++j) {
                u32x4 o;
#pragma unroll
                for (int e = 0; e < 4; ++e)
                    o[e] = pack_bf2(lrelu1((sum[m][j][2 * e] + 0.f) * a.inv_n, a.slope), lrelu1((sum[m][j][2 * e + 1] + 0.f) * a.inv_n, a.slope));
                __builtin_amdgcn_raw_buffer_store_b128(o, yr, (int)pvoff[m][j], 0, 0);
            }
    }
}

struct PairTile { int WT, WC, MT, NT, MINB, M; };

inline bool pair_tile_for(int C, PairTile* t) {
    if (C == 32) {
        *t = PairTile{4, 1, 3, 1, 4, 384};
        return true;
    }
    if (C == 64) {
        *t = PairTile{2, 2, 4, 1, 3, 256};
        return true;
    }
    if (C == 128) { *t = PairTile{2, 2, 3, 2, 2, 192}; return true; }
    return false;
}

inline bool pair_applicable(const PairLaunch& a, int nz) {
    PairTile t;
    if (nz < 1 || nz > kMaxGroup || !pair_tile_for(a.C, &t)) return false;
    if (!(a.slope >= 0.f && a.slope <= 1.f)) return false;
    if ((double)a.L * a.C * 2.0 >= 2147483648.0) return false;
    for (int j = 0; j < nz; ++j) {
        const int ks = a.p[j].ks, d = a.p[j].dil;
        if (ks < 1 || !(ks & 1) || d < 1) return false;
        if (ks - 1 >= t.M / 2) return false;
        if ((ks - 1) * d > kPairSpanMax) return false;
        if ((size_t)(t.M + (ks - 1) * d) * (a.C * 2 + 16) > 66 * 1024) return false;
    }
    return true;
}

inline hipError_t launch_pair_bf16(PairLaunch& a, int nz, hipStream_t stream) {
    PairTile t;
    if (!pair_tile_for(a.C, &t)) return hipErrorInvalidValue;
    for (int j = 0; j < nz; ++j)
        for (int i = 0; i < nz; ++i)
            if (a.p[j].x == a.p[i].y) return hipErrorInvalidValue;
    a.nz = nz;
    a.Qp = packed_qsteps(a.C);
    a.n_ct = packed_cotiles(a.C);
    int span = 0, kmax = 1;
    for (int j = 0; j < nz; ++j) {
        const int s = (a.p[j].ks - 1) * a.p[j].dil;
        if (s > span) span = s;
        if (a.p[j].ks > kmax) kmax = a.p[j].ks;
    }
    const int t_out_min = t.M - (kmax - 1);
    const long long tiles = (a.L + t_out_min - 1) / t_out_min;
    const long long n_jobs = tiles * nz;
    if (n_jobs > 0x3fffffffLL || a.B > 65535) return hipErrorInvalidValue;
    a.n_jobs = (int)n_jobs;
    a.jobs_per_xcd = (int)((n_jobs + 7) / 8);
    const size_t window_bytes = (size_t)(t.M + span) * (a.C * 2 + 16);
    const size_t scratch_bytes = (size_t)4 * 32 * (t.NT * 32 * 4 + 16);
    const size_t lds_bytes = window_bytes > scratch_bytes ? window_bytes : scratch_bytes;
    dim3 grid((unsigned)(a.jobs_per_xcd * 8), (unsigned)a.B, 1u), block(256);
#define IRIS_PAIR_CASE(WT_, WC_, MT_, NT_, C_, MINB_)                                                        \
    if (a.C == C_ && t.WT == WT_ && t.WC == WC_ && t.MT == MT_ && t.NT == NT_ && t.MINB == MINB_) {        \
        auto kfn = mrf_pair_bf16_kernel<WT_, WC_, MT_, NT_, C_, MINB_>;                                      \
        { const hipError_t e__ = ::iris::launch_kernel_named("mrf_pair_bf16_kernel", kfn, grid, block, lds_bytes, stream, a); if (e__ != hipSuccess) return e__; } \
        return hipSuccess;                                                                                   \
    }
    IRIS_PAIR_CASE(4, 1, 3, 1, 32, 4)
    IRIS_PAIR_CASE(2, 2, 4, 1, 64, 3)
    IRIS_PAIR_CASE(2, 2, 3, 2, 128, 2)
#undef IRIS_PAIR_CASE
    return hipErrorInvalidValue;
}

inline bool pair_sum_tile_for(int C, PairTile* t) {
    if (C == 32)  { *t = PairTile{4, 1, IRIS_B16_SUM32_MT, 1, IRIS_B16_SUM32_MINB, 4 * IRIS_B16_SUM32_MT * 32}; return true; }
    if (C == 64)  { *t = PairTile{2, 2, IRIS_B16_SUM64_MT, 1, IRIS_B16_SUM64_MINB, 2 * IRIS_B16_SUM64_MT * 32}; return true; }
    return false;
}

inline bool pair_sum_applicable(const PairLaunch& a, int nz, bool f32_out) {
    PairTile t;
    if (nz != 3 || !pair_sum_tile_for(a.C, &t)) return false;
    if (!(a.slope >= 0.f && a.slope <= 1.f)) return false;
    if ((double)a.L * a.C * (f32_out ? 4.0 : 2.0) >= 2147483648.0) return false;
    for (int j = 0; j < nz; ++j) {
        const int ks = a.p[j].ks, d = a.p[j].dil;
        if (ks < 1 || !(ks & 1) || d < 1) return false;
        if (ks - 1 >= t.M / 2) return false;
        if ((ks - 1) * d > kPairSpanMax) return false;
        if ((size_t)(t.M + (ks - 1) * d) * (a.C * 2 + 16) > 66 * 1024) return false;
    }
    return IRIS_B16_PAIR_SUM_DEFAULT != 0;
}

inline hipError_t launch_pair_bf16_sum(PairLaunch& a, void* sum_y, bool f32_out, hipStream_t stream) {
    PairTile t;
    if (!pair_sum_tile_for(a.C, &t) || !sum_y) return hipErrorInvalidValue;
    for (int j = 0; j < 3; ++j)
        if ((const void*)a.p[j].x == sum_y) return hipErrorInvalidValue;
    a.nz = 3;
    a.Qp = packed_qsteps(a.C);
    a.n_ct = packed_cotiles(a.C);
    a.sum_y = sum_y; a.sum_f32 = f32_out ? 1 : 0; a.inv_n = 1.0f / 3.0f;
    int span = 0, kmax = 1;
    for (int j = 0; j < 3; ++j) {
        const int s = (a.p[j].ks - 1) * a.p[j].dil;
        if (s > span) span = s;
        if (a.p[j].ks > kmax) kmax = a.p[j].ks;
    }
    const int t_out = t.M - (kmax - 1);
    const long long tiles = (a.L + t_out - 1) / t_out;
    if (tiles > 0x3fffffffLL || a.B > 65535) return hipErrorInvalidValue;
    a.n_jobs = (int)tiles;
    a.jobs_per_xcd = (int)((tiles + 7) / 8);
    const size_t window_bytes = (size_t)(t.M + span) * (a.C * 2 + 16);
    const size_t scratch_bytes = (size_t)4 * 32 * (t.NT * 32 * 4 + 16);
    const size_t lds_bytes = window_bytes > scratch_bytes ? window_bytes : scratch_bytes;
    dim3 grid((unsigned)(a.jobs_per_xcd * 8), (unsigned)a.B, 1u), block(256);
#define IRIS_PAIR_SUM_CASE(WT_, WC_, MT_, NT_, C_, MINB_)                                                    \
    if (a.C == C_ && t.WT == WT_ && t.WC == WC_ && t.MT == MT_ && t.NT == NT_ && t.MINB == MINB_) {        \
        auto kfn = mrf_pair_bf16_sum_kernel<WT_, WC_, MT_, NT_, C_, MINB_>;                                  \
        { const hipError_t e__ = ::iris::launch_kernel_named("mrf_pair_bf16_sum_kernel", kfn, grid, block, lds_bytes, stream, a); if (e__ != hipSuccess) return e__; } \
        return hipSuccess;                                                                                   \
    }
    IRIS_PAIR_SUM_CASE(4, 1, IRIS_B16_SUM32_MT, 1, 32, IRIS_B16_SUM32_MINB)
    IRIS_PAIR_SUM_CASE(2, 2, IRIS_B16_SUM64_MT, 1, 64, IRIS_B16_SUM64_MINB)
#undef IRIS_PAIR_SUM_CASE
    return hipErrorInvalidValue;
}

}
}
```

Measured before the change: 53.34 million.

## Switch bf16 conv kernels from 32x32x16 to 16x16x32 MFMA with a two-deep weight ring

The bf16 conv, transposed-conv and resblock kernels now use the 16x16x32 bf16 MFMA instead of 32x32x16. Accumulators are split into 16x16 fragments, and the weight packing order on the host is changed to match, with a selectable fragment order so the f32-split path keeps the old layout. Weight prefetch becomes a shared two-deep ring with a tail guard, replacing the per-kernel depth of 2 or 4. The aim is better MFMA throughput and shorter dependency chains, at the cost of more instructions per K step and a shallower prefetch.

```diff
diff --git a/iris-tts_amd/csrc/conv_mfma_bf16.h b/iris-tts_amd/csrc/conv_mfma_bf16.h
--- a/iris-tts_amd/csrc/conv_mfma_bf16.h
+++ b/iris-tts_amd/csrc/conv_mfma_bf16.h
@@ -176,53 +176,96 @@
     }
 }
 
+#ifndef IRIS_B16_RING_TAIL_GUARD
+#define IRIS_B16_RING_TAIL_GUARD 1
+#endif
+constexpr int kRing = 2;
+
+template <int CIC>
+__device__ __forceinline__ unsigned w_group_soff(int n, unsigned q_bytes, unsigned tap_bytes) {
+    constexpr int QPC = CIC / 32;
+    constexpr int QL = QPC == 4 ? 2 : (QPC == 2 ? 1 : 0);
+    static_assert(QPC == 4 || QPC == 2 || QPC == 1, "CIC must be 32, 64 or 128");
+    return (unsigned)(n >> QL) * tap_bytes + (unsigned)(n & (QPC - 1)) * q_bytes;
+}
+
+template <int NT, int CIC>
+__device__ __forceinline__ void ring_request(u32x4 (&wv)[kRing][2 * NT], __amdgpu_buffer_rsrc_t wr, unsigned wvoff,
+                                             unsigned q_bytes, unsigned tap_bytes, unsigned q0_bytes) {
+#pragma unroll
+    for (int i = 0; i < kRing; ++i) {
+#pragma unroll
+        for (int f = 0; f < 2 * NT; ++f)
+            wv[i][f] = buf_load4(wr, wvoff + (unsigned)f * 1024u, q0_bytes + w_group_soff<CIC>(i, q_bytes, tap_bytes));
+        __builtin_amdgcn_sched_barrier(0);
+    }
+}
+
 template <int MT, int NT, int CIC>
-__device__ __forceinline__ void mma_chunk(f32x16 (&acc)[MT][NT], const char* a_lane, int dil_bytes,
-                                          __amdgpu_buffer_rsrc_t wr, unsigned wvoff, unsigned q_bytes,
-                                          unsigned tap_bytes, unsigned q0_bytes, int ks) {
-    constexpr int QPC = CIC / 16;
-    constexpr int QL = QPC == 8 ? 3 : (QPC == 4 ? 2 : (QPC == 2 ? 1 : 0));
-    static_assert(QPC == 8 || QPC == 4 || QPC == 2 || QPC == 1, "CIC must be 16, 32, 64 or 128");
+__device__ __forceinline__ void ring_mma_loop(f32x4 (&acc)[2 * MT][2 * NT], u32x4 (&wv)[kRing][2 * NT], const char* a_lane,
+                                              int dil_bytes, __amdgpu_buffer_rsrc_t wr, unsigned wvoff, unsigned q_bytes,
+                                              unsigned tap_bytes, unsigned q0_bytes, int ks) {
+    constexpr int QPC = CIC / 32;
+    constexpr int QL = QPC == 4 ? 2 : (QPC == 2 ? 1 : 0);
     constexpr int SB = CIC * 2 + 16;
-    constexpr int D = (QPC == 2 && MT * NT >= 8) ? 2 : 4;
     const int NG = ks * QPC;
-    auto w_soff = [&](int n) -> unsigned {
-        return (unsigned)(n >> QL) * tap_bytes + q0_bytes + (unsigned)(n & (QPC - 1)) * q_bytes;
-    };
-    auto load_a = [&](u32x4 (&av)[MT], int n) {
+    auto load_a = [&](u32x4 (&av)[MT], int n, int rh) {
         int tap = n >> QL;
         tap = tap < ks ? tap : ks - 1;
-        const char* ap = a_lane + tap * dil_bytes + (n & (QPC - 1)) * 32;
+        const char* ap = a_lane + tap * dil_bytes + (n & (QPC - 1)) * 64 + rh * 16 * SB;
 #pragma unroll
         for (int m = 0; m < MT; ++m) av[m] = *reinterpret_cast<const u32x4*>(ap + m * 32 * SB);
     };
-    u32x4 wv[D][NT], av[2][MT];
-#pragma unroll
-    for (int i = 0; i < D; ++i) {
-#pragma unroll
-        for (int nt = 0; nt < NT; ++nt) wv[i][nt] = buf_load4(wr, wvoff + (unsigned)nt * 1024u, w_soff(i));
-        __builtin_amdgcn_sched_barrier(0);
-    }
-    load_a(av[0], 0);
-    for (int n0 = 0; n0 < NG; n0 += D) {
-#pragma unroll
-        for (int i = 0; i < D; ++i) {
-            const int n = n0 + i;
-            load_a(av[(i + 1) & 1], n + 1);
+    u32x4 av[2][MT];
+    load_a(av[0], 0, 0);
+    auto group = [&](int i, int n) {
+#pragma unroll
+        for (int rh = 0; rh < 2; ++rh) {
+            load_a(av[rh ^ 1], n + rh, rh ^ 1);
             __builtin_amdgcn_sched_barrier(0);
 #pragma unroll
-            for (int nt = 0; nt < NT; ++nt)
+            for (int f = 0; f < 2 * NT; ++f)
 #pragma unroll
                 for (int m = 0; m < MT; ++m)
-                    acc[m][nt] = __builtin_amdgcn_mfma_f32_32x32x16_bf16(
-                        __builtin_bit_cast(bf16x8, wv[i][nt]), __builtin_bit_cast(bf16x8, av[i & 1][m]),
-                        acc[m][nt], 0, 0, 0);
+                    acc[2 * m + rh][f] = __builtin_amdgcn_mfma_f32_16x16x32_bf16(
+                        __builtin_bit_cast(bf16x8, wv[i][f]), __builtin_bit_cast(bf16x8, av[rh][m]), acc[2 * m + rh][f], 0, 0, 0);
             __builtin_amdgcn_sched_barrier(0);
-#pragma unroll
-            for (int nt = 0; nt < NT; ++nt)
-                wv[i][nt] = buf_load4(wr, wvoff + (unsigned)nt * 1024u, w_soff(n + D));
-        }
-    }
+        }
+#pragma unroll
+        for (int f = 0; f < 2 * NT; ++f)
+            wv[i][f] = buf_load4(wr, wvoff + (unsigned)f * 1024u, q0_bytes + w_group_soff<CIC>(n + kRing, q_bytes, tap_bytes));
+    };
+    constexpr bool kTail = IRIS_B16_RING_TAIL_GUARD && (QPC % kRing) != 0;
+    const int NG_main = kTail ? (NG / kRing) * kRing : NG;
+    int n0 = 0;
+    for (; n0 < NG_main; n0 += kRing) {
+#pragma unroll
+        for (int i = 0; i < kRing; ++i) group(i, n0 + i);
+    }
+    if constexpr (kTail) {
+        if (n0 < NG) group(0, n0);
+    }
+}
+
+template <int MT, int NT>
+__device__ __forceinline__ void acc_from_bias(f32x4 (&acc)[2 * MT][2 * NT], const float* bias, int co0, int kg, int cmax) {
+#pragma unroll
+    for (int f = 0; f < 2 * NT; ++f) {
+        const int co = co0 + 16 * f + 4 * kg;
+        const f32x4 b4 = *reinterpret_cast<const f32x4*>(bias + (co < cmax ? co : 0));
+#pragma unroll
+        for (int m = 0; m < 2 * MT; ++m) acc[m][f] = b4;
+    }
+}
+
+template <int MT, int NT>
+__device__ __forceinline__ void acc_to_scratch(const f32x4 (&acc)[2 * MT][2 * NT], int m, char* scr, int l15, int kg) {
+    constexpr int RS = NT * 32 * 4 + 16;
+#pragma unroll
+    for (int rh = 0; rh < 2; ++rh)
+#pragma unroll
+        for (int f = 0; f < 2 * NT; ++f)
+            *reinterpret_cast<f32x4*>(scr + (rh * 16 + l15) * RS + (f * 16 + 4 * kg) * 4) = acc[2 * m + rh][f];
 }
 
 template <int WT, int WC, int MT, int NT, int CIC, int MINB>
@@ -233,7 +276,7 @@
     constexpr int T_BLK = WT * MT * 32;
     const int lane = threadIdx.x & 63, wave = threadIdx.x >> 6;
     const int wt = wave / WC, wc = wave - wt * WC;
-    const int lo = lane & 31, hi = lane >> 5;
+    const int l15 = lane & 15, kg = lane >> 4;
 
     int w_item, sub;
     int b = blockIdx.y;
@@ -268,34 +311,27 @@
     const int ct0 = (tile_co * WC + wc) * NT;
     const bool wave_active = ct0 < a.n_ct;
 
-    f32x16 acc[MT][NT];
-#pragma unroll
-    for (int nt = 0; nt < NT; ++nt)
-#pragma unroll
-        for (int g = 0; g < 4; ++g) {
-            const int co = (ct0 + nt) * 32 + 8 * g + 4 * hi;
-            const f32x4 b4 = *reinterpret_cast<const f32x4*>(p.bias + (co < a.C_out ? co : 0));
-#pragma unroll
-            for (int m = 0; m < MT; ++m)
-#pragma unroll
-                for (int e = 0; e < 4; ++e) acc[m][nt][4 * g + e] = b4[e];
-        }
-
-    const unsigned q_bytes = (unsigned)a.n_ct * 1024u;
-    const unsigned tap_bytes = (unsigned)a.Qp * q_bytes;
+    f32x4 acc[2 * MT][2 * NT];
+    acc_from_bias<MT, NT>(acc, p.bias, ct0 * 32, kg, a.C_out);
+
+    const unsigned q_bytes = (unsigned)a.n_ct * 2048u;
+    const unsigned tap_bytes = (unsigned)a.Qp * (unsigned)a.n_ct * 1024u;
     const char* wbase = (const char*)p.wp + (a.z_is_phase ? (size_t)z * a.phase_wp_bytes : 0);
     const __amdgpu_buffer_rsrc_t wr = make_rsrc(wbase, (unsigned)ks * tap_bytes);
-    const unsigned wvoff = (unsigned)ct0 * 1024u + (unsigned)lane * 16u;
-    const char* a_lane = lds + (wt * MT * 32 + lo) * SB + hi * 16;
+    const unsigned wvoff = (unsigned)ct0 * 2048u + (unsigned)lane * 16u;
+    const char* a_lane = lds + (wt * MT * 32 + l15) * SB + kg * 16;
     const int dil_bytes = p.dil * SB;
 
     for (int c0 = 0; c0 < a.C_in; c0 += CIC) {
         if (c0 > 0) __syncthreads();
         stage_window<CIC>(a, p, lds, b, in_row0, R, c0);
         __syncthreads();
-        if (wave_active)
-            mma_chunk<MT, NT, CIC>(acc, a_lane, dil_bytes, wr, wvoff, q_bytes, tap_bytes,
-                                   (unsigned)(c0 >> 4) * q_bytes, ks);
+        if (wave_active) {
+            const unsigned q0_bytes = (unsigned)(c0 >> 5) * q_bytes;
+            u32x4 wv[kRing][2 * NT];
+            ring_request<NT, CIC>(wv, wr, wvoff, q_bytes, tap_bytes, q0_bytes);
+            ring_mma_loop<MT, NT, CIC>(acc, wv, a_lane, dil_bytes, wr, wvoff, q_bytes, tap_bytes, q0_bytes, ks);
+        }
     }
     __syncthreads();
     if (!wave_active) return;
@@ -330,15 +366,7 @@
         for (int j = 0; j < NP; ++j) resv[m][j] = buf_load4(rr, pvoff[m][j], 0);
 #pragma unroll
     for (int m = 0; m < MT; ++m) {
-#pragma unroll
-        for (int nt = 0; nt < NT; ++nt)
-#pragma unroll
-            for (int g = 0; g < 4; ++g) {
-                f32x4 v;
-#pragma unroll
-                for (int e = 0; e < 4; ++e) v[e] = acc[m][nt][4 * g + e];
-                *reinterpret_cast<f32x4*>(scr + lo * RS + (nt * 32 + 8 * g + 4 * hi) * 4) = v;
-            }
+        acc_to_scratch<MT, NT>(acc, m, scr, l15, kg);
         __builtin_amdgcn_fence(__ATOMIC_RELEASE, "wavefront");
         __builtin_amdgcn_wave_barrier();
         __builtin_amdgcn_fence(__ATOMIC_ACQUIRE, "wavefront");
@@ -452,47 +480,56 @@
     return (uint16_t)(u >> 16);
 }
 
+enum FragOrder : int { FRAG_16x16x32 = 0, FRAG_32x32x16 = 1 };
+inline void frag_coords(FragOrder order, int t, int n_ct, int lane, int e, int* co, int* ci) {
+    if (order == FRAG_16x16x32) {
+        const int g = t / (2 * n_ct), ct16 = t - g * 2 * n_ct;
+        *co = 16 * ct16 + (lane & 15);
+        *ci = 32 * g + 8 * (lane >> 4) + e;
+    } else {
+        const int q = t / n_ct, ct = t - q * n_ct;
+        *co = 32 * ct + (lane & 31);
+        *ci = 16 * q + 8 * (lane >> 5) + e;
+    }
+}
 inline int packed_qsteps(int C_in) { return ((C_in + 63) / 64) * 4; }
 inline int packed_cotiles(int C_out) { return (C_out + 31) / 32; }
 inline size_t packed_conv1d_halfs(int C_in, int C_out, int ks) {
     return (size_t)ks * packed_qsteps(C_in) * packed_cotiles(C_out) * 64 * 8;
 }
-inline void pack_conv1d_bf16(const float* w, int C_in, int C_out, int ks, uint16_t* out) {
+inline void pack_conv1d_bf16(const float* w, int C_in, int C_out, int ks, uint16_t* out, FragOrder order = FRAG_16x16x32) {
     const int Qp = packed_qsteps(C_in), n_ct = packed_cotiles(C_out);
     for (int kap = 0; kap < ks; ++kap)
-        for (int q = 0; q < Qp; ++q)
-            for (int ct = 0; ct < n_ct; ++ct)
-                for (int lane = 0; lane < 64; ++lane)
-                    for (int e = 0; e < 8; ++e) {
-                        const int co = ct * 32 + (lane & 31);
-                        const int ci = 16 * q + 8 * (lane >> 5) + e;
-                        float v = 0.f;
-                        if (co < C_out && ci < C_in) v = w[((size_t)co * C_in + ci) * ks + kap];
-                        out[((((size_t)kap * Qp + q) * n_ct + ct) * 64 + lane) * 8 + e] = f32_to_bf16(v);
-                    }
+        for (int t = 0; t < Qp * n_ct; ++t)
+            for (int lane = 0; lane < 64; ++lane)
+                for (int e = 0; e < 8; ++e) {
+                    int co, ci;
+                    frag_coords(order, t, n_ct, lane, e, &co, &ci);
+                    float v = 0.f;
+                    if (co < C_out && ci < C_in) v = w[((size_t)co * C_in + ci) * ks + kap];
+                    out[(((size_t)kap * Qp * n_ct + t) * 64 + lane) * 8 + e] = f32_to_bf16(v);
+                }
 }
 inline int convt_taps(int k, int u) { return (k + u - 1) / u; }
 inline size_t packed_convt_phase_halfs(int C_in, int C_out, int k, int u) {
     return packed_conv1d_halfs(C_in, C_out, convt_taps(k, u));
 }
-inline void pack_convt_bf16(const float* w, int C_in, int C_out, int k, int u, uint16_t* out) {
+inline void pack_convt_bf16(const float* w, int C_in, int C_out, int k, int u, uint16_t* out, FragOrder order = FRAG_16x16x32) {
     const int taps = convt_taps(k, u);
     const int Qp = packed_qsteps(C_in), n_ct = packed_cotiles(C_out);
     const size_t phase_halfs = packed_convt_phase_halfs(C_in, C_out, k, u);
     for (int ph = 0; ph < u; ++ph)
         for (int kap = 0; kap < taps; ++kap) {
             const int kk = ph + (taps - 1 - kap) * u;
-            for (int q = 0; q < Qp; ++q)
-                for (int ct = 0; ct < n_ct; ++ct)
-                    for (int lane = 0; lane < 64; ++lane)
-                        for (int e = 0; e < 8; ++e) {
-                            const int co = ct * 32 + (lane & 31);
-                            const int ci = 16 * q + 8 * (lane >> 5) + e;
-                            float v = 0.f;
-                            if (co < C_out && ci < C_in && kk < k) v = w[((size_t)ci * C_out + co) * k + kk];
-                            out[ph * phase_halfs + ((((size_t)kap * Qp + q) * n_ct + ct) * 64 + lane) * 8 + e] =
-                                f32_to_bf16(v);
-                        }
+            for (int t = 0; t < Qp * n_ct; ++t)
+                for (int lane = 0; lane < 64; ++lane)
+                    for (int e = 0; e < 8; ++e) {
+                        int co, ci;
+                        frag_coords(order, t, n_ct, lane, e, &co, &ci);
+                        float v = 0.f;
+                        if (co < C_out && ci < C_in && kk < k) v = w[((size_t)ci * C_out + co) * k + kk];
+                        out[ph * phase_halfs + (((size_t)kap * Qp * n_ct + t) * 64 + lane) * 8 + e] = f32_to_bf16(v);
+                    }
         }
 }
 
diff --git a/iris-tts_amd/csrc/conv_mfma_f32s.h b/iris-tts_amd/csrc/conv_mfma_f32s.h
--- a/iris-tts_amd/csrc/conv_mfma_f32s.h
+++ b/iris-tts_amd/csrc/conv_mfma_f32s.h
@@ -292,8 +292,8 @@
         hi[i] = hf;
         mid[i] = w[i] - hf;
     }
-    b16::pack_conv1d_bf16(hi.data(), C_in, C_out, ks, out);
-    b16::pack_conv1d_bf16(mid.data(), C_in, C_out, ks, out + packed_plane_halfs(C_in, C_out, ks));
+    b16::pack_conv1d_bf16(hi.data(), C_in, C_out, ks, out, b16::FRAG_32x32x16);
+    b16::pack_conv1d_bf16(mid.data(), C_in, C_out, ks, out + packed_plane_halfs(C_in, C_out, ks), b16::FRAG_32x32x16);
 }
 
 inline size_t packed_convt_plane_halfs(int C_in, int C_out, int k, int u) { return b16::packed_convt_phase_halfs(C_in, C_out, k, u) * u; }
@@ -308,8 +308,8 @@
         hi[i] = hf;
         mid[i] = w[i] - hf;
     }
-    b16::pack_convt_bf16(hi.data(), C_in, C_out, k, u, out);
-    b16::pack_convt_bf16(mid.data(), C_in, C_out, k, u, out + packed_convt_plane_halfs(C_in, C_out, k, u));
+    b16::pack_convt_bf16(hi.data(), C_in, C_out, k, u, out, b16::FRAG_32x32x16);
+    b16::pack_convt_bf16(mid.data(), C_in, C_out, k, u, out + packed_convt_plane_halfs(C_in, C_out, k, u), b16::FRAG_32x32x16);
 }
 
 struct Tile { int WT, WC, MT, NT, CIC, MINB, T_BLK, CO_BLK; };
diff --git a/iris-tts_amd/csrc/convt_mfma_bf16.h b/iris-tts_amd/csrc/convt_mfma_bf16.h
--- a/iris-tts_amd/csrc/convt_mfma_bf16.h
+++ b/iris-tts_amd/csrc/convt_mfma_bf16.h
@@ -39,14 +39,15 @@
     char* const lds = lds_b16;
     constexpr int SB = CIC * 2 + 16;
     constexpr int PPR = CIC / 8;
-    constexpr int QPC = CIC / 16;
+    constexpr int QPC = CIC / 32;
     constexpr int R_BLK = WR * MT * 32;
     constexpr int WIN = R_BLK + 1;
     constexpr int NQ = (WIN * PPR + 255) / 256;
     constexpr int RPI = 256 / PPR;
     constexpr int NG = 2 * QPC;
-    constexpr int LPG = (NQ + NG - 1) / NG;
-    constexpr int DB = 4;
+    constexpr int NS = 2 * NG;
+    constexpr int LPG = (NQ + NS - 1) / NS;
+    constexpr int DB = kRing;
     static_assert(DB <= QPC && NG > DB, "the ring reaches into tap 0 of the next phase only");
     constexpr int RS = NT * 32 * 4 + 16;
     constexpr int PPRO = NT * 4;
@@ -54,14 +55,14 @@
 
     const int tid = threadIdx.x, lane = tid & 63, wave = tid >> 6;
     const int wr = wave / WC, wc = wave - wr * WC;
-    const int lo = lane & 31, hi = lane >> 5;
+    const int l15 = lane & 15, kg = lane >> 4;
     const int C = a.C_in;
     const int n_chunks = C / CIC;
     const float slope = a.in_act == IN_ACT_NONE ? 1.f : a.slope;
     const unsigned in_bytes = (unsigned)a.L_in * (unsigned)C * 2u;
     const unsigned out_bytes = (unsigned)a.L_out * (unsigned)a.C_out * 2u;
-    const unsigned q_bytes = (unsigned)a.n_ct * 1024u;
-    const unsigned tap_bytes = (unsigned)a.Qp * q_bytes;
+    const unsigned q_bytes = (unsigned)a.n_ct * 2048u;
+    const unsigned tap_bytes = (unsigned)a.Qp * (unsigned)a.n_ct * 1024u;
     const __amdgpu_buffer_rsrc_t wrs = make_rsrc(a.wp, (unsigned)a.u * a.phase_bytes);
     char* const scr = lds + WIN * SB + wave * (32 * RS);
     float* const lds_bias = reinterpret_cast<float*>(lds + WIN * SB + 4 * (32 * RS));
@@ -101,7 +102,7 @@
             }
     };
 
-    struct Tile { size_t x_off, y_off; int i0, gct0; unsigned wvoff[NT]; };
+    struct Tile { size_t x_off, y_off; int i0, gct0; unsigned wvoff[2 * NT]; };
     const int xmul = a.xcd_order ? 8 : 1;
     const int xcd = a.xcd_order ? (int)(blockIdx.x & 7) : 0;
     const int slot = a.xcd_order ? (int)(blockIdx.x >> 3) : (int)blockIdx.x;
@@ -120,14 +121,15 @@
         for (int nt = 0; nt < NT; ++nt) {
             const int gct = t.gct0 + nt;
             const int ph = gct / a.n_ct, ct = gct - ph * a.n_ct;
-            t.wvoff[nt] = (unsigned)ph * a.phase_bytes + (unsigned)(ct * 64 + lane) * 16u;
+            t.wvoff[2 * nt] = (unsigned)ph * a.phase_bytes + (unsigned)(ct * 128 + lane) * 16u;
+            t.wvoff[2 * nt + 1] = t.wvoff[2 * nt] + 1024u;
         }
         return t;
     };
 
-    const char* a_lane = lds + (wr * MT * 32 + lo) * SB + hi * 16;
-    f32x16 acc[MT][NT];
-    u32x4 bw[DB + 1][NT];
+    const char* a_lane = lds + (wr * MT * 32 + l15) * SB + kg * 16;
+    f32x4 acc[2 * MT][2 * NT];
+    u32x4 bw[DB + 1][2 * NT];
 
     int job = slot;
     if (!job_valid(job)) return;
@@ -139,7 +141,7 @@
 #pragma unroll
         for (int d = 0; d < DB; ++d)
 #pragma unroll
-            for (int nt = 0; nt < NT; ++nt) bw[d][nt] = buf_load4(wrs, t.wvoff[nt], (unsigned)d * q_bytes);
+            for (int f = 0; f < 2 * NT; ++f) bw[d][f] = buf_load4(wrs, t.wvoff[f], (unsigned)d * q_bytes);
         stage_write_all();
         __syncthreads();
     }
@@ -152,12 +154,10 @@
             const int gct = t.gct0 + nt;
             const int ct = gct % a.n_ct;
 #pragma unroll
-            for (int g = 0; g < 4; ++g) {
-                const f32x4 b4 = *reinterpret_cast<const f32x4*>(lds_bias + ct * 32 + 8 * g + 4 * hi);
-#pragma unroll
-                for (int m = 0; m < MT; ++m)
-#pragma unroll
-                    for (int e = 0; e < 4; ++e) acc[m][nt][4 * g + e] = b4[e];
+            for (int ch = 0; ch < 2; ++ch) {
+                const f32x4 b4 = *reinterpret_cast<const f32x4*>(lds_bias + ct * 32 + 16 * ch + 4 * kg);
+#pragma unroll
+                for (int m = 0; m < 2 * MT; ++m) acc[m][2 * nt + ch] = b4;
             }
         }
 
@@ -170,46 +170,49 @@
             const unsigned vbn = stage_vbase(tq.i0 - 1, cq * CIC);
             const unsigned wsoff0 = (unsigned)(chunk * QPC) * q_bytes;
             const unsigned wsoffn = (unsigned)(cq * QPC) * q_bytes;
-            auto a_ptr = [&](int n) { return a_lane + (n / QPC) * SB + (n % QPC) * 32; };
-            auto b_load = [&](int n, int nt) {
+            auto a_ptr = [&](int s) { return a_lane + ((s >> 1) / QPC) * SB + ((s >> 1) % QPC) * 64 + (s & 1) * 16 * SB; };
+            auto b_load = [&](int n, int f) {
                 if (n < NG)
-                    return buf_load4(wrs, t.wvoff[nt], wsoff0 + (unsigned)(n / QPC) * tap_bytes + (unsigned)(n % QPC) * q_bytes);
-                return buf_load4(wrs, has_next ? tq.wvoff[nt] : kOob, wsoffn + (unsigned)(n - NG) * q_bytes);
+                    return buf_load4(wrs, t.wvoff[f], wsoff0 + (unsigned)(n / QPC) * tap_bytes + (unsigned)(n % QPC) * q_bytes);
+                return buf_load4(wrs, has_next ? tq.wvoff[f] : kOob, wsoffn + (unsigned)(n - NG) * q_bytes);
             };
             u32x4 av[2][MT];
 #pragma unroll
             for (int m = 0; m < MT; ++m) av[0][m] = *reinterpret_cast<const u32x4*>(a_ptr(0) + m * 32 * SB);
 #pragma unroll
-            for (int n = 0; n < NG; ++n) {
+            for (int s = 0; s < NS; ++s) {
+                const int n = s >> 1, rh = s & 1;
 #pragma unroll
                 for (int l = 0; l < LPG; ++l)
-                    if (n * LPG + l < NQ) stage_load_one(n * LPG + l, tq.x_off, in_bytes_n, vbn);
-#pragma unroll
-                for (int nt = 0; nt < NT; ++nt) bw[(n + DB) % (DB + 1)][nt] = b_load(n + DB, nt);
-                if (n + 1 < NG) {
+                    if (s * LPG + l < NQ) stage_load_one(s * LPG + l, tq.x_off, in_bytes_n, vbn);
+                if (rh == 0) {
+#pragma unroll
+                    for (int f = 0; f < 2 * NT; ++f) bw[(n + DB) % (DB + 1)][f] = b_load(n + DB, f);
+                }
+                if (s + 1 < NS) {
 #pragma unroll
                     for (int m = 0; m < MT; ++m)
-                        av[(n + 1) & 1][m] = *reinterpret_cast<const u32x4*>(a_ptr(n + 1) + m * 32 * SB);
-                }
-#pragma unroll
-                for (int nt = 0; nt < NT; ++nt)
+                        av[(s + 1) & 1][m] = *reinterpret_cast<const u32x4*>(a_ptr(s + 1) + m * 32 * SB);
+                }
+#pragma unroll
+                for (int f = 0; f < 2 * NT; ++f)
 #pragma unroll
                     for (int m = 0; m < MT; ++m)
-                        acc[m][nt] = __builtin_amdgcn_mfma_f32_32x32x16_bf16(
-                            __builtin_bit_cast(bf16x8, bw[n % (DB + 1)][nt]), __builtin_bit_cast(bf16x8, av[n & 1][m]),
-                            acc[m][nt], 0, 0, 0);
+                        acc[2 * m + rh][f] = __builtin_amdgcn_mfma_f32_16x16x32_bf16(
+                            __builtin_bit_cast(bf16x8, bw[n % (DB + 1)][f]), __builtin_bit_cast(bf16x8, av[s & 1][m]),
+                            acc[2 * m + rh][f], 0, 0, 0);
                 __builtin_amdgcn_sched_barrier(0);
             }
             {
-                u32x4 tmp[DB][NT];
+                u32x4 tmp[DB][2 * NT];
 #pragma unroll
                 for (int d = 0; d < DB; ++d)
 #pragma unroll
-                    for (int nt = 0; nt < NT; ++nt) tmp[d][nt] = bw[(NG + d) % (DB + 1)][nt];
+                    for (int f = 0; f < 2 * NT; ++f) tmp[d][f] = bw[(NG + d) % (DB + 1)][f];
 #pragma unroll
                 for (int d = 0; d < DB; ++d)
 #pragma unroll
-                    for (int nt = 0; nt < NT; ++nt) bw[d][nt] = tmp[d][nt];
+                    for (int f = 0; f < 2 * NT; ++f) bw[d][f] = tmp[d][f];
             }
             if (last) {
                 const __amdgpu_buffer_rsrc_t yr = make_rsrc(a.y + t.y_off, out_bytes);
@@ -225,15 +228,7 @@
                 }
 #pragma unroll
                 for (int m = 0; m < MT; ++m) {
-#pragma unroll
-                    for (int nt = 0; nt < NT; ++nt)
-#pragma unroll
-                        for (int g = 0; g < 4; ++g) {
-                            f32x4 v;
-#pragma unroll
-                            for (int e = 0; e < 4; ++e) v[e] = acc[m][nt][4 * g + e];
-                            *reinterpret_cast<f32x4*>(scr + lo * RS + (nt * 32 + 8 * g + 4 * hi) * 4) = v;
-                        }
+                    acc_to_scratch<MT, NT>(acc, m, scr, l15, kg);
                     __builtin_amdgcn_fence(__ATOMIC_RELEASE, "wavefront");
                     __builtin_amdgcn_wave_barrier();
                     __builtin_amdgcn_fence(__ATOMIC_ACQUIRE, "wavefront");
diff --git a/iris-tts_amd/csrc/mrf_pair_bf16.h b/iris-tts_amd/csrc/mrf_pair_bf16.h
--- a/iris-tts_amd/csrc/mrf_pair_bf16.h
+++ b/iris-tts_amd/csrc/mrf_pair_bf16.h
@@ -5,9 +5,6 @@
 #define IRIS_B16_RES_EARLY 1
 #endif
 
-#ifndef IRIS_B16_RING_TAIL_GUARD
-#define IRIS_B16_RING_TAIL_GUARD 1
-#endif
 #ifndef IRIS_B16_PAIR_SUM_DEFAULT
 #define IRIS_B16_PAIR_SUM_DEFAULT 1
 #endif
@@ -56,67 +53,6 @@
 
 __device__ __forceinline__ float lrelu_max(float v, float slope) { return fmaxf(v, v * slope); }
 
-template <int NT, int CIC, int D>
-__device__ __forceinline__ void ring_request(u32x4 (&wv)[D][NT], __amdgpu_buffer_rsrc_t wr, unsigned wvoff,
-                                             unsigned q_bytes, unsigned tap_bytes) {
-    constexpr int QPC = CIC / 16;
-    constexpr int QL = QPC == 8 ? 3 : (QPC == 4 ? 2 : (QPC == 2 ? 1 : 0));
-#pragma unroll
-    for (int i = 0; i < D; ++i) {
-#pragma unroll
-        for (int nt = 0; nt < NT; ++nt)
-            wv[i][nt] = buf_load4(wr, wvoff + (unsigned)nt * 1024u, (unsigned)(i >> QL) * tap_bytes + (unsigned)(i & (QPC - 1)) * q_bytes);
-        __builtin_amdgcn_sched_barrier(0);
-    }
-}
-
-template <int MT, int NT, int CIC, int D>
-__device__ __forceinline__ void ring_mma_loop(f32x16 (&acc)[MT][NT], u32x4 (&wv)[D][NT], const char* a_lane, int dil_bytes,
-                                              __amdgpu_buffer_rsrc_t wr, unsigned wvoff, unsigned q_bytes,
-                                              unsigned tap_bytes, int ks) {
-    constexpr int QPC = CIC / 16;
-    constexpr int QL = QPC == 8 ? 3 : (QPC == 4 ? 2 : (QPC == 2 ? 1 : 0));
-    constexpr int SB = CIC * 2 + 16;
-    const int NG = ks * QPC;
-    auto w_soff = [&](int n) -> unsigned { return (unsigned)(n >> QL) * tap_bytes + (unsigned)(n & (QPC - 1)) * q_bytes; };
-    auto load_a = [&](u32x4 (&av)[MT], int n) {
-        int tap = n >> QL;
-        tap = tap < ks ? tap : ks - 1;
-        const char* ap = a_lane + tap * dil_bytes + (n & (QPC - 1)) * 32;
-#pragma unroll
-        for (int m = 0; m < MT; ++m) av[m] = *reinterpret_cast<const u32x4*>(ap + m * 32 * SB);
-    };
-    u32x4 av[2][MT];
-    load_a(av[0], 0);
-    auto group = [&](int i, int n) {
-        load_a(av[(i + 1) & 1], n + 1);
-        __builtin_amdgcn_sched_barrier(0);
-#pragma unroll
-        for (int nt = 0; nt < NT; ++nt)
-#pragma unroll
-            for (int m = 0; m < MT; ++m)
-                acc[m][nt] = __builtin_amdgcn_mfma_f32_32x32x16_bf16(
-                    __builtin_bit_cast(bf16x8, wv[i][nt]), __builtin_bit_cast(bf16x8, av[i & 1][m]), acc[m][nt], 0, 0, 0);
-        __builtin_amdgcn_sched_barrier(0);
-#pragma unroll
-        for (int nt = 0; nt < NT; ++nt)
-            wv[i][nt] = buf_load4(wr, wvoff + (unsigned)nt * 1024u, w_soff(n + D));
-    };
-    constexpr bool kTail = IRIS_B16_RING_TAIL_GUARD && (QPC % D) != 0;
-    const int NG_main = kTail ? (NG / D) * D : NG;
-    int n0 = 0;
-    for (; n0 < NG_main; n0 += D) {
-#pragma unroll
-        for (int i = 0; i < D; ++i) group(i, n0 + i);
-    }
-    if constexpr (kTail) {
-        if (n0 < NG) {
-#pragma unroll
-            for (int i = 0; i < QPC; ++i) group(i, n0 + i);
-        }
-    }
-}
-
 template <int WT, int WC, int MT, int NT, int C, int MINB>
 __global__ void __launch_bounds__(256, MINB) mrf_pair_bf16_kernel(const PairLaunch a) {
     extern __shared__ __attribute__((aligned(16))) char lds_pair[];
@@ -126,10 +62,9 @@
     constexpr int M = WT * MT * 32;
     constexpr int PPR = C / 8;
     constexpr int NQ = ((M + kPairSpanMax) * PPR + 255) / 256;
-    constexpr int D = 4;
     const int lane = threadIdx.x & 63, wave = threadIdx.x >> 6;
     const int wt = wave / WC, wc = wave - wt * WC;
-    const int lo = lane & 31, hi = lane >> 5;
+    const int l15 = lane & 15, kg = lane >> 4;
 
     const int xcd = blockIdx.x & 7, slot = blockIdx.x >> 3;
     const int job = xcd * a.jobs_per_xcd + slot;
@@ -151,28 +86,24 @@
 
     const unsigned tensor_bytes = (unsigned)L * (unsigned)C * 2u;
     const size_t item = (size_t)b * L * C;
-    const unsigned q_bytes = (unsigned)a.n_ct * 1024u;
-    const unsigned tap_bytes = (unsigned)a.Qp * q_bytes;
-    const unsigned wvoff = (unsigned)ct0 * 1024u + (unsigned)lane * 16u;
-    const char* a_lane = lds + (wt * MT * 32 + lo) * SB + hi * 16;
+    const unsigned q_bytes = (unsigned)a.n_ct * 2048u;
+    const unsigned tap_bytes = (unsigned)a.Qp * (unsigned)a.n_ct * 1024u;
+    const unsigned wvoff = (unsigned)ct0 * 2048u + (unsigned)lane * 16u;
+    const char* a_lane = lds + (wt * MT * 32 + l15) * SB + kg * 16;
     const __amdgpu_buffer_rsrc_t xr = make_rsrc(p.x + item, tensor_bytes);
     const __amdgpu_buffer_rsrc_t wr1 = make_rsrc(p.w1, (unsigned)ks * tap_bytes);
     const __amdgpu_buffer_rsrc_t wr2 = make_rsrc(p.w2, (unsigned)ks * tap_bytes);
 
-    f32x16 acc[MT][NT];
-    auto load_bias = [&](f32x4 (&bias4)[NT][4], const float* bptr) {
-#pragma unroll
-        for (int nt = 0; nt < NT; ++nt)
-#pragma unroll
-            for (int g = 0; g < 4; ++g) bias4[nt][g] = *reinterpret_cast<const f32x4*>(bptr + (ct0 + nt) * 32 + 8 * g + 4 * hi);
+    f32x4 acc[2 * MT][2 * NT];
+    auto load_bias = [&](f32x4 (&bias4)[2 * NT], const float* bptr) {
+#pragma unroll
+        for (int f = 0; f < 2 * NT; ++f) bias4[f] = *reinterpret_cast<const f32x4*>(bptr + ct0 * 32 + 16 * f + 4 * kg);
     };
-    auto init_acc = [&](const f32x4 (&bias4)[NT][4]) {
-#pragma unroll
-        for (int m = 0; m < MT; ++m)
-#pragma unroll
-            for (int nt = 0; nt < NT; ++nt)
-#pragma unroll
-                for (int r = 0; r < 16; ++r) acc[m][nt][r] = bias4[nt][r >> 2][r & 3];
+    auto init_acc = [&](const f32x4 (&bias4)[2 * NT]) {
+#pragma unroll
+        for (int m = 0; m < 2 * MT; ++m)
+#pragma unroll
+            for (int f = 0; f < 2 * NT; ++f) acc[m][f] = bias4[f];
     };
 
     constexpr int RS = NT * 32 * 4 + 16;
@@ -200,10 +131,10 @@
     constexpr int RBUF = IRIS_B16_RES_EARLY ? MT : 2;
     u32x4 resv[RBUF][NP];
     if constexpr (IRIS_B16_RES_EARLY) geometry(lane);
-    f32x4 bias4[NT][4];
+    f32x4 bias4[2 * NT];
     load_bias(bias4, p.b1);
-    u32x4 wv[D][NT];
-    ring_request<NT, C, D>(wv, wr1, wvoff, q_bytes, tap_bytes);
+    u32x4 wv[kRing][2 * NT];
+    ring_request<NT, C>(wv, wr1, wvoff, q_bytes, tap_bytes, 0u);
     {
         const int in_row0 = o0 - h2 - h1, R = M + (ks - 1) * dil, total = R * PPR;
         u32x4 v[NQ];
@@ -236,27 +167,25 @@
     }
     __syncthreads();
     init_acc(bias4);
-    ring_mma_loop<MT, NT, C, D>(acc, wv, a_lane, dil * SB, wr1, wvoff, q_bytes, tap_bytes, ks);
-    ring_request<NT, C, D>(wv, wr2, wvoff, q_bytes, tap_bytes);
+    ring_mma_loop<MT, NT, C>(acc, wv, a_lane, dil * SB, wr1, wvoff, q_bytes, tap_bytes, 0u, ks);
+    ring_request<NT, C>(wv, wr2, wvoff, q_bytes, tap_bytes, 0u);
     load_bias(bias4, p.b2);
     __syncthreads();
 #pragma unroll
-    for (int m = 0; m < MT; ++m) {
-        const int row_l = (wt * MT + m) * 32 + lo;
+    for (int m = 0; m < 2 * MT; ++m) {
+        const int row_l = wt * MT * 32 + m * 16 + l15;
         const int row_g = o0 - h2 + row_l;
         const unsigned keep = (row_g >= 0 && row_g < L) ? 0xffffffffu : 0u;
 #pragma unroll
-        for (int nt = 0; nt < NT; ++nt)
-#pragma unroll
-            for (int g = 0; g < 4; ++g) {
-                u32x2 o;
-#pragma unroll
-                for (int e2 = 0; e2 < 2; ++e2) {
-                    const unsigned t = pack_bf2(acc[m][nt][4 * g + 2 * e2], acc[m][nt][4 * g + 2 * e2 + 1]);
-                    o[e2] = pack_bf2(lrelu_max(bf_lo(t), a.slope), lrelu_max(bf_hi(t), a.slope)) & keep;
-                }
-                *reinterpret_cast<u32x2*>(lds + row_l * SB + ((ct0 + nt) * 32 + 8 * g + 4 * hi) * 2) = o;
-            }
+        for (int f = 0; f < 2 * NT; ++f) {
+            u32x2 o;
+#pragma unroll
+            for (int e2 = 0; e2 < 2; ++e2) {
+                const unsigned t = pack_bf2(acc[m][f][2 * e2], acc[m][f][2 * e2 + 1]);
+                o[e2] = pack_bf2(lrelu_max(bf_lo(t), a.slope), lrelu_max(bf_hi(t), a.slope)) & keep;
+            }
+            *reinterpret_cast<u32x2*>(lds + row_l * SB + (ct0 * 32 + 16 * f + 4 * kg) * 2) = o;
+        }
     }
     {
         int lane2 = lane;
@@ -269,7 +198,7 @@
     }
     __syncthreads();
     init_acc(bias4);
-    ring_mma_loop<MT, NT, C, D>(acc, wv, a_lane, SB, wr2, wvoff, q_bytes, tap_bytes, ks);
+    ring_mma_loop<MT, NT, C>(acc, wv, a_lane, SB, wr2, wvoff, q_bytes, tap_bytes, 0u, ks);
     __syncthreads();
     char* scr = lds + wave * (32 * RS);
 #pragma unroll
@@ -278,15 +207,7 @@
 #pragma unroll
             for (int j = 0; j < NP; ++j) resv[(m + 1) & 1][j] = buf_load4(rr, pvoff[m + 1][j], 0);
         }
-#pragma unroll
-        for (int nt = 0; nt < NT; ++nt)
-#pragma unroll
-            for (int g = 0; g < 4; ++g) {
-                f32x4 v;
-#pragma unroll
-                for (int e = 0; e < 4; ++e) v[e] = acc[m][nt][4 * g + e];
-                *reinterpret_cast<f32x4*>(scr + lo * RS + (nt * 32 + 8 * g + 4 * hi) * 4) = v;
-            }
+        acc_to_scratch<MT, NT>(acc, m, scr, l15, kg);
         __builtin_amdgcn_fence(__ATOMIC_RELEASE, "wavefront");
         __builtin_amdgcn_wave_barrier();
         __builtin_amdgcn_fence(__ATOMIC_ACQUIRE, "wavefront");
@@ -323,11 +244,10 @@
     constexpr int M = WT * MT * 32;
     constexpr int PPR = C / 8;
     constexpr int NQ = ((M + kPairSpanMax) * PPR + 255) / 256;
-    constexpr int D = 4;
     constexpr int NZ = 3;
     const int lane = threadIdx.x & 63, wave = threadIdx.x >> 6;
     const int wt = wave / WC, wc = wave - wt * WC;
-    const int lo = lane & 31, hi = lane >> 5;
+    const int l15 = lane & 15, kg = lane >> 4;
     const int xcd = blockIdx.x & 7, slot = blockIdx.x >> 3;
     const int tile = xcd * a.jobs_per_xcd + slot;
     if (tile >= a.n_jobs) return;
@@ -342,10 +262,10 @@
     const int ct0 = wc * NT;
     const unsigned tensor_bytes = (unsigned)L * (unsigned)C * 2u;
     const size_t item = (size_t)b * L * C;
-    const unsigned q_bytes = (unsigned)a.n_ct * 1024u;
-    const unsigned tap_bytes = (unsigned)a.Qp * q_bytes;
-    const unsigned wvoff = (unsigned)ct0 * 1024u + (unsigned)lane * 16u;
-    const char* a_lane = lds + (wt * MT * 32 + lo) * SB + hi * 16;
+    const unsigned q_bytes = (unsigned)a.n_ct * 2048u;
+    const unsigned tap_bytes = (unsigned)a.Qp * (unsigned)a.n_ct * 1024u;
+    const unsigned wvoff = (unsigned)ct0 * 2048u + (unsigned)lane * 16u;
+    const char* a_lane = lds + (wt * MT * 32 + l15) * SB + kg * 16;
 
     constexpr int RS = NT * 32 * 4 + 16;
     constexpr int PPRO = NT * 4;
@@ -366,20 +286,16 @@
         }
     }
     float sum[MT][NP][8];
-    f32x16 acc[MT][NT];
-    auto load_bias = [&](f32x4 (&bias4)[NT][4], const float* bptr) {
-#pragma unroll
-        for (int nt = 0; nt < NT; ++nt)
-#pragma unroll
-            for (int g = 0; g < 4; ++g) bias4[nt][g] = *reinterpret_cast<const f32x4*>(bptr + (ct0 + nt) * 32 + 8 * g + 4 * hi);
+    f32x4 acc[2 * MT][2 * NT];
+    auto load_bias = [&](f32x4 (&bias4)[2 * NT], const float* bptr) {
+#pragma unroll
+        for (int f = 0; f < 2 * NT; ++f) bias4[f] = *reinterpret_cast<const f32x4*>(bptr + ct0 * 32 + 16 * f + 4 * kg);
     };
-    auto init_acc = [&](const f32x4 (&bias4)[NT][4]) {
-#pragma unroll
-        for (int m = 0; m < MT; ++m)
-#pragma unroll
-            for (int nt = 0; nt < NT; ++nt)
-#pragma unroll
-                for (int r = 0; r < 16; ++r) acc[m][nt][r] = bias4[nt][r >> 2][r & 3];
+    auto init_acc = [&](const f32x4 (&bias4)[2 * NT]) {
+#pragma unroll
+        for (int m = 0; m < 2 * MT; ++m)
+#pragma unroll
+            for (int f = 0; f < 2 * NT; ++f) acc[m][f] = bias4[f];
     };
     char* scr = lds + wave * (32 * RS);
 
@@ -393,10 +309,10 @@
         const __amdgpu_buffer_rsrc_t wr1 = make_rsrc(p.w1, (unsigned)ks * tap_bytes);
         const __amdgpu_buffer_rsrc_t wr2 = make_rsrc(p.w2, (unsigned)ks * tap_bytes);
         if (z > 0) __syncthreads();
-        f32x4 bias4[NT][4];
+        f32x4 bias4[2 * NT];
         load_bias(bias4, p.b1);
-        u32x4 wv[D][NT];
-        ring_request<NT, C, D>(wv, wr1, wvoff, q_bytes, tap_bytes);
+        u32x4 wv[kRing][2 * NT];
+        ring_request<NT, C>(wv, wr1, wvoff, q_bytes, tap_bytes, 0u);
         {
             const int in_row0 = o0 - h2 - h1, R = M + (ks - 1) * dil, total = R * PPR;
             u32x4 v[NQ];
@@ -423,27 +339,25 @@
         }
         __syncthreads();
         init_acc(bias4);
-        ring_mma_loop<MT, NT, C, D>(acc, wv, a_lane, dil * SB, wr1, wvoff, q_bytes, tap_bytes, ks);
-        ring_request<NT, C, D>(wv, wr2, wvoff, q_bytes, tap_bytes);
+        ring_mma_loop<MT, NT, C>(acc, wv, a_lane, dil * SB, wr1, wvoff, q_bytes, tap_bytes, 0u, ks);
+        ring_request<NT, C>(wv, wr2, wvoff, q_bytes, tap_bytes, 0u);
         load_bias(bias4, p.b2);
         __syncthreads();
 #pragma unroll
-        for (int m = 0; m < MT; ++m) {
-            const int row_l = (wt * MT + m) * 32 + lo;
+        for (int m = 0; m < 2 * MT; ++m) {
+            const int row_l = wt * MT * 32 + m * 16 + l15;
             const int row_g = o0 - h2 + row_l;
             const unsigned keep = (row_g >= 0 && row_g < L) ? 0xffffffffu : 0u;
 #pragma unroll
-            for (int nt = 0; nt < NT; ++nt)
-#pragma unroll
-                for (int g = 0; g < 4; ++g) {
-                    u32x2 o;
-#pragma unroll
-                    for (int e2 = 0; e2 < 2; ++e2) {
-                        const unsigned t = pack_bf2(acc[m][nt][4 * g + 2 * e2], acc[m][nt][4 * g + 2 * e2 + 1]);
-                        o[e2] = pack_bf2(lrelu_max(bf_lo(t), a.slope), lrelu_max(bf_hi(t), a.slope)) & keep;
-                    }
-                    *reinterpret_cast<u32x2*>(lds + row_l * SB + ((ct0 + nt) * 32 + 8 * g + 4 * hi) * 2) = o;
+            for (int f = 0; f < 2 * NT; ++f) {
+                u32x2 o;
+#pragma unroll
+                for (int e2 = 0; e2 < 2; ++e2) {
+                    const unsigned t = pack_bf2(acc[m][f][2 * e2], acc[m][f][2 * e2 + 1]);
+                    o[e2] = pack_bf2(lrelu_max(bf_lo(t), a.slope), lrelu_max(bf_hi(t), a.slope)) & keep;
                 }
+                *reinterpret_cast<u32x2*>(lds + row_l * SB + (ct0 * 32 + 16 * f + 4 * kg) * 2) = o;
+            }
         }
         const __amdgpu_buffer_rsrc_t rr = make_rsrc(p.x + item, tensor_bytes);
         constexpr int RB = (MT * NT > 3) ? 1 : 2;
@@ -454,7 +368,7 @@
         }
         __syncthreads();
         init_acc(bias4);
-        ring_mma_loop<MT, NT, C, D>(acc, wv, a_lane, SB, wr2, wvoff, q_bytes, tap_bytes, ks);
+        ring_mma_loop<MT, NT, C>(acc, wv, a_lane, SB, wr2, wvoff, q_bytes, tap_bytes, 0u, ks);
         __syncthreads();
 #pragma unroll
         for (int m = 0; m < MT; ++m) {
@@ -467,15 +381,7 @@
 #pragma unroll
                 for (int j = 0; j < NP; ++j) resv[0][j] = buf_load4(rr, pvoff[m][j], 0);
             }
-#pragma unroll
-            for (int nt = 0; nt < NT; ++nt)
-#pragma unroll
-                for (int g = 0; g < 4; ++g) {
-                    f32x4 v;
-#pragma unroll
-                    for (int e = 0; e < 4; ++e) v[e] = acc[m][nt][4 * g + e];
-                    *reinterpret_cast<f32x4*>(scr + lo * RS + (nt * 32 + 8 * g + 4 * hi) * 4) = v;
-                }
+            acc_to_scratch<MT, NT>(acc, m, scr, l15, kg);
             __builtin_amdgcn_fence(__ATOMIC_RELEASE, "wavefront");
             __builtin_amdgcn_wave_barrier();
             __builtin_amdgcn_fence(__ATOMIC_ACQUIRE, "wavefront");
```

After: 53.37 million, median of 2. About the same (+0.1%).
